# servo/webrender

Measured on AMD Instinct MI355X. Metric: frames/sec + Mpixels/sec on wrench benchmarks, 4K target, 1/2/4/8 GPU, higher is better.
Workload: dtype u8; 1 GPU; cfg2: 1000 overlapping translucent rects (ps_quad_textured + premultiplied-alpha blend), 3840x2160, 20 picture-cache tiles + composite, seed 2; encoding=quad, target=3840x2160, parallelism=single GPU

## Files before the change

include/wrhip.h:

```cpp
#ifndef WRHIP_H
#define WRHIP_H

#include <stddef.h>
#include <stdint.h>

#ifdef __cplusplus
extern "C" {
#endif

typedef int8_t GLbyte;
typedef uint8_t GLubyte;
typedef int16_t GLshort;
typedef uint16_t GLushort;
typedef int32_t GLint;
typedef uint32_t GLuint;
typedef int64_t GLint64;
typedef uint64_t GLuint64;
typedef float GLfloat;
typedef double GLdouble;
typedef uint32_t GLenum;
typedef uint8_t GLboolean;
typedef uint32_t GLbitfield;
typedef int32_t GLsizei;
typedef size_t GLsizeiptr;
// ... 97 lines not shown
                GLenum ty, void* data);
void Finish(void);
void ShaderSourceByName(GLuint shader, const GLchar* name);
void TexParameteri(GLenum target, GLenum pname, GLint param);
void CopyImageSubData(GLuint src_name, GLenum src_target, GLint src_level,
                      GLint src_x, GLint src_y, GLint src_z, GLuint dst_name,
                      GLenum dst_target, GLint dst_level, GLint dst_x,
                      GLint dst_y, GLint dst_z, GLsizei src_width,
                      GLsizei src_height, GLsizei src_depth);
void CopyTexSubImage2D(GLenum target, GLint level, GLint xoffset, GLint yoffset,
                       GLint x, GLint y, GLsizei width,
                       GLsizei height);
void BlitFramebuffer(GLint src_x0, GLint src_y0, GLint src_x1, GLint src_y1,
                     GLint dst_x0, GLint dst_y0, GLint dst_x1, GLint dst_y1,
                     GLbitfield mask, GLenum filter);
void GetIntegerv(GLenum pname, GLint* params);
void GetBooleanv(GLenum pname, GLboolean* params);
const char* GetString(GLenum name);
const char* GetStringi(GLenum name, GLuint index);
GLenum GetError(void);
void InitDefaultFramebuffer(int32_t x, int32_t y, int32_t width, int32_t height,
                            int32_t stride, void* buf);
void* GetColorBuffer(GLuint fbo, GLboolean flush, int32_t* width,
                     int32_t* height, int32_t* stride);
void ResolveFramebuffer(GLuint fbo);
void SetTextureBuffer(GLuint tex, GLenum internal_format, GLsizei width,
                      GLsizei height, GLsizei stride, void* buf,
                      GLsizei min_width, GLsizei min_height);
void SetTextureParameter(GLuint tex, GLenum pname, GLint param);
void DeleteTexture(GLuint n);
void DeleteRenderbuffer(GLuint n);
void DeleteFramebuffer(GLuint n);
void DeleteBuffer(GLuint n);
void DeleteVertexArray(GLuint n);
void DeleteQuery(GLuint n);
void DeleteShader(GLuint shader);
void DeleteProgram(GLuint program);
LockedTexture* LockFramebuffer(GLuint fbo);
LockedTexture* LockTexture(GLuint tex);
void LockResource(LockedTexture* resource);
void UnlockResource(LockedTexture* resource);
void* GetResourceBuffer(LockedTexture* resource, int32_t* width,
                        int32_t* height, int32_t* stride);
void Composite(LockedTexture* locked_dst, LockedTexture* locked_src, GLint src_x,
               GLint src_y, GLsizei src_width, GLsizei src_height, GLint dst_x,
               GLint dst_y, GLsizei dst_width, GLsizei dst_height,
               GLboolean opaque, GLboolean flip_x, GLboolean flip_y,
               GLenum filter, GLint clip_x, GLint clip_y, GLsizei clip_width,
               GLsizei clip_height);
void CompositeYUV(LockedTexture* locked_dst, LockedTexture* locked_y,
                  LockedTexture* locked_u, LockedTexture* locked_v,
                  YuvRangedColorSpace color_space, GLuint color_depth,
                  GLint src_x, GLint src_y, GLsizei src_width,
                  GLsizei src_height, GLint dst_x, GLint dst_y,
                  GLsizei dst_width, GLsizei dst_height, GLboolean flip_x,
                  GLboolean flip_y, GLint clip_x, GLint clip_y,
                  GLsizei clip_width, GLsizei clip_height);
WrhipContext* CreateContext(void);
void ReferenceContext(WrhipContext* ctx);
void DestroyContext(WrhipContext* ctx);
void MakeCurrent(WrhipContext* ctx);
size_t ReportMemory(WrhipContext* ctx,
                    size_t (*size_of_op)(const void* ptr));


typedef struct WrhipStats {
  uint64_t flushes;
  uint64_t kernel_launches;
  uint64_t raster_launches;
  uint64_t raster_ns;
  uint64_t raster_algo_bytes;
  uint64_t raster_pixels;
  uint64_t prims;
  uint64_t h2d_bytes;
  uint64_t d2h_bytes;
  uint64_t host_record_ns;
  uint64_t host_upload_ns;
  uint64_t host_flush_ns;
  uint64_t host_wait_ns;
  uint64_t row_launches;
  uint64_t setup_carried;
  uint64_t carrier_lost;
  uint64_t scratch_grown_held;
} WrhipStats;
void WrhipGetStats(WrhipStats* out);
void WrhipResetStats(void);
void WrhipSetProfiling(int enabled);
typedef struct WrhipKernelStat {
  int32_t kind, fmt, depth, feat;
  uint64_t launches, ns, algo_bytes, workgroups;
} WrhipKernelStat;
int32_t WrhipGetKernelStats(WrhipKernelStat* out, int32_t max);
void WrhipSetShard(int rank, int world);
void WrhipSetTargetRows(GLuint tex, int32_t y0, int32_t y1);
void* WrhipGetTextureDevicePtr(GLuint tex, int32_t* width, int32_t* height,
                               int32_t* stride);
GLuint WrhipGetFramebufferTexture(GLuint fbo);
const char* WrhipDeviceName(void);
void WrhipFlush(void);
int WrhipFlushHeld(void);
void* WrhipGetStream(void);

#ifdef __cplusplus
}
#endif
#endif
```

webrender_amd/csrc/wrhip.hip:

```cpp
#include <vector>
#include <map>
#include <algorithm>
#include <time.h>
#include <chrono>
#include <thread>
#include <pthread.h>
#include <mutex>
#include <condition_variable>
#include <atomic>
#include <functional>

#include "../../include/wrhip.h"
#include "wrhip_glenum.h"
#include "wrhip_types.h"
#include "wrhip_rt.h"
#include "wrhip_kernels.h"
#ifndef WRHIP_HOSTSIM
#include "wrhip_inst.h"
#define WR_INST_DECLARE(K, SIG, ...) extern template __global__ void K<__VA_ARGS__> SIG;
WR_INST_ALL(WR_INST_DECLARE)
#undef WR_INST_DECLARE
#endif

namespace {
// ... 325 lines not shown
  int sampler_unit[WR_MAX_TEX];
  float transform[16];
  Program() {
    for (int& a : attrib_loc) a = NULL_ATTRIB;
    for (int& s : sampler_unit) s = 0;
    memset(transform, 0, sizeof(transform));
  }
};

struct TargetWork {
  GLuint tex = 0;
  GLuint depth_tex = 0;
  std::vector<WrDrawDesc> draws;
  std::vector<uint8_t> inst;
  std::vector<GLuint> reads;
  std::vector<GLuint> rreads;
  int prims = 0;
  int level = 0;
  uint32_t init_depth = 0xFFFFFF;
  bool init_depth_set = false, depth_live = false;
  GLuint fwd_tex = 0; int fwd_dx = 0, fwd_y0 = 0, fwd_ys = 1, fwd_clip[4] = {0, 0, 0, 0};
  bool forwarded_away = false;
  void recycle() {
    std::vector<WrDrawDesc> d; d.swap(draws); d.clear();
    std::vector<uint8_t> i; i.swap(inst); i.clear();
    std::vector<GLuint> r; r.swap(reads); r.clear();
    std::vector<GLuint> rr; rr.swap(rreads); rr.clear();
    *this = TargetWork();
    draws.swap(d); inst.swap(i); reads.swap(r); rreads.swap(rr);
  }
};

const size_t MAX_TEXTURE_UNITS = 16;

struct Context {
  int32_t references = 1;
  ObjectStore<Query> queries;
  ObjectStore<Buffer> buffers;
  ObjectStore<Texture> textures;
  ObjectStore<VertexArray> vertex_arrays;
  ObjectStore<Framebuffer> framebuffers;
  ObjectStore<Renderbuffer> renderbuffers;
  ObjectStore<Shader> shaders;
  ObjectStore<Program> programs;

  GLenum last_error = GL_NO_ERROR;
  int viewport[4] = {0, 0, 0, 0};
  bool blend = false;
  GLenum blendfunc_srgb = GL_ONE, blendfunc_drgb = GL_ZERO, blendfunc_sa = GL_ONE, blendfunc_da = GL_ZERO;
  GLenum blend_equation = GL_FUNC_ADD;
  uint32_t blendcolor[2] = {0, 0};
  int blend_key = WR_BLEND_NONE;
  bool depthtest = false, depthmask = true;
  GLenum depthfunc = GL_LESS;
  bool scissortest = false;
  int scissor[4] = {0, 0, 0, 0};
  float clearcolor[4] = {0, 0, 0, 0};
  double cleardepth = 1;
  int unpack_row_length = 0;

  struct TextureUnit { GLuint texture_2d_binding = 0, texture_rectangle_binding = 0; };
  TextureUnit texture_units[MAX_TEXTURE_UNITS];
  int active_texture_unit = 0;
  GLuint current_program = 0, current_vertex_array = 0;
  GLuint pixel_pack_buffer_binding = 0, pixel_unpack_buffer_binding = 0, array_buffer_binding = 0;
  GLuint time_elapsed_query = 0, samples_passed_query = 0;
  GLuint renderbuffer_binding = 0, draw_framebuffer_binding = 0, read_framebuffer_binding = 0;
  GLuint unknown_binding = 0;

  wr_stream_t stream;
  std::vector<TargetWork> work;
  std::vector<TargetWork> spare;
  std::vector<GLuint> referenced;
  struct UploadSeg { uint64_t src_off; void* dst; uint32_t dst_stride, row_bytes, rows, pad; };
  std::vector<UploadSeg> useg;
  size_t upload_begin = 0;
  bool upload_open = false;
  uint64_t lap_ns[8] = {0, 0, 0, 0, 0, 0, 0, 0}; uint64_t lap_n = 0;
  uint64_t upload_batch = 1;
  bool scatter_first = false;
  std::vector<GLuint> view_texs;
  struct PendingScatter { size_t seg_off = 0; int nseg = 0, parts = 0; uint64_t bytes = 0; bool valid = false; } ps;
  bool fuse_scatter = true;
  uint8_t* dupload = nullptr;
  struct Scratch {
    WrPrim* prims = nullptr; size_t prims_cap = 0;
    WrRec* recs = nullptr;
    WrAux* aux = nullptr;
    float* vtab = nullptr; size_t vtab_cap = 0;
    float* qtab = nullptr; size_t qtab_cap = 0;
    unsigned long long* masks = nullptr; size_t masks_cap = 0;
    unsigned* bin_ctr = nullptr; size_t bin_ctr_cap = 0;
    unsigned long long* mr_ctl = nullptr; WrMaskSlot* mr_slots = nullptr; size_t mr_slots_cap = 0;
    uint8_t* mr_store = nullptr; size_t mr_store_cap = 0;
    unsigned long long mr_seen = 0;
    uint32_t* flat = nullptr; size_t flat_cap = 0;
  } scratch[2];
  int64_t flush_seq = 0;
  int64_t held_seq = 0;
  int fb_writes_since_held = 0;
  bool last_flush_wrote_fb = false;
  struct Held { int fmt, depth, feat, nb, off; uint64_t algo_bytes; int mr_rows = 0; int dense = 0; int row_t0 = 0, row_n = 0, row_items = 0, row_mode = 0; };
  struct Tail {
    bool pending = false;
    std::vector<Held> held;
    int n_targets = 0;
    const WrTargetDesc* targets = nullptr; const WrDrawDesc* draws = nullptr;
    int set = 0;
    std::vector<GLuint> refs;
  } tail;
  bool defer_tail = true;
  wr_stream_t copy_stream;
  wr_event_t ev_copy;
  bool copy_overlap = true;
  wr_stream_t setup_stream;
  wr_event_t ev_up, ev_setup;
  bool setup_on_stream = false;
  WrUnsupportedCounters* dcounters = nullptr;
  WrUnsupportedCounters seen = {};
  std::multimap<size_t, void*> pool;
  size_t pool_bytes = 0;
  uint8_t* staging = nullptr; size_t staging_size = 0, staging_pos = 0;
  uint64_t ring_base = 0, ring_safe = 0;
  struct RingFence { uint64_t v = 0; wr_event_t ev; bool made = false; };
  static const int RING_FENCES = 8;
  RingFence ring_fence[RING_FENCES];
  uint64_t ring_fences = 0;
  bool profiling = false;
  bool profiling_deferred = false;
  wr_event_t ev_a, ev_b;
  WrhipStats stats;
  std::vector<WrhipKernelStat> kstats;
  int shard_rank = 0, shard_world = 1;
  int next_query_slot = 0;
  GLuint query_slot_owner[WR_QUERY_SLOTS] = {};
  bool forward_composites = true;
  bool profiling_no_forward = false;
  bool mask_rows = true;
  bool span_rows = true;
  bool tile_rows = true;
  bool grad_tables = true;
  size_t gtab_pending = 0;
  bool quad_rowtabs = true;
  size_t runs_pool_words = (size_t)16 << 20;
  unsigned long long* last_qctl = nullptr;
  size_t last_qtab_cap = 0;
  uint64_t last_qctl_v = 0;
  bool cell_raster = true;
  bool thin_r8 = true;
  int thin_parts = 4;
  bool dense_text = false;
  int chain_grid = 0;
  unsigned chain_base = 0;

  Context() {
    wrrt::stream_create(&stream);
    wrrt::stream_create(&copy_stream);
    wrrt::event_create_sync(&ev_copy);
    wrrt::stream_create(&setup_stream);
    wrrt::event_create_sync(&ev_up);
    wrrt::event_create_sync(&ev_setup);
    setup_on_stream = getenv("WRHIP_SETUP_STREAM") && atoi(getenv("WRHIP_SETUP_STREAM")) != 0;
    copy_overlap = getenv("WRHIP_NO_COPY_STREAM") == nullptr;
    forward_composites = getenv("WRHIP_NO_FORWARD") == nullptr;
    thin_r8 = getenv("WRHIP_NO_THIN") == nullptr;
    if (const char* e = getenv("WRHIP_THIN_PARTS")) { const int v = atoi(e); if (v == 1 || v == 2 || v == 4 || v == 8 || v == 16) thin_parts = v; }
    dense_text = getenv("WRHIP_DENSE_TEXT") != nullptr;
    if (thin_r8 && getenv("WRHIP_CHAIN") && atoi(getenv("WRHIP_CHAIN")) > 0)
      chain_grid = getenv("WRHIP_CHAIN_GRID") ? atoi(getenv("WRHIP_CHAIN_GRID")) : wrrt::cu_count() / 2;
    cell_raster = getenv("WRHIP_NO_CELLS") == nullptr;
    fuse_scatter = getenv("WRHIP_NO_FUSE_SCATTER") == nullptr;
    mask_rows = getenv("WRHIP_NO_MASK_ROWS") == nullptr;
    span_rows = getenv("WRHIP_NO_SPAN_ROWS") == nullptr;
    tile_rows = getenv("WRHIP_NO_TILE_ROWS") == nullptr;
    quad_rowtabs = getenv("WRHIP_NO_QTAB") == nullptr;
    grad_tables = getenv("WRHIP_NO_GTAB") == nullptr;
    if (const char* e = getenv("WRHIP_RUNS_POOL_WORDS")) runs_pool_words = (size_t)atoll(e);
    wrrt::event_create(&ev_a); wrrt::event_create(&ev_b);
    memset(&stats, 0, sizeof(stats));
    dcounters = (WrUnsupportedCounters*)wrrt::dev_alloc(sizeof(WrUnsupportedCounters));
    wrrt::memset8(dcounters, 0, sizeof(WrUnsupportedCounters), stream);
  }
  ~Context();

  GLuint& get_binding(GLenum name) {
    switch (name) {
      case GL_PIXEL_PACK_BUFFER: return pixel_pack_buffer_binding;
      case GL_PIXEL_UNPACK_BUFFER: return pixel_unpack_buffer_binding;
      case GL_ARRAY_BUFFER: return array_buffer_binding;
      case GL_ELEMENT_ARRAY_BUFFER: return vertex_arrays[current_vertex_array].element_array_buffer_binding;
      case GL_TEXTURE_2D: return texture_units[active_texture_unit].texture_2d_binding;
      case GL_TEXTURE_RECTANGLE: return texture_units[active_texture_unit].texture_rectangle_binding;
      case GL_TIME_ELAPSED: return time_elapsed_query;
      case GL_SAMPLES_PASSED: return samples_passed_query;
      case GL_RENDERBUFFER: return renderbuffer_binding;
      case GL_DRAW_FRAMEBUFFER: return draw_framebuffer_binding;
      case GL_READ_FRAMEBUFFER: return read_framebuffer_binding;
      default: return unknown_binding;
    }
  }
};

Context* ctx = nullptr;
bool g_rt_ok = false, g_rt_tried = false;
char g_device_name[256] = "";

void ensure_runtime() {
  if (g_rt_tried) {
    if (!g_rt_ok) { fprintf(stderr, "libwrhip: no HIP device available; this backend has no CPU path\n"); abort(); }
    return;
  }
  g_rt_tried = true;
  int dev = 0;
  g_rt_ok = wrrt::init(&dev, g_device_name, sizeof(g_device_name));
  if (!g_rt_ok) { fprintf(stderr, "libwrhip: no HIP device available; this backend has no CPU path\n"); abort(); }
}

int bytes_for_internal_format(GLenum f) {
  switch (f) {
    case GL_RGBA32F: case GL_RGBA32I: return 16;
    case GL_RGBA8: case GL_BGRA8: case GL_RGBA: return 4;
    case GL_R8: case GL_RED: return 1;
    case GL_RG8: case GL_RG: return 2;
    case GL_DEPTH_COMPONENT: case GL_DEPTH_COMPONENT16: case GL_DEPTH_COMPONENT24: case GL_DEPTH_COMPONENT32: return 4;
    case GL_RGB_RAW_422_APPLE: return 2;
    case GL_R16: return 2;
    case GL_RG16: return 4;
    default: return 0;
  }
}
int aligned_stride(int row_bytes) { return (row_bytes + 3) & ~3; }
GLenum remap_internal_format(GLenum format) {
  switch (format) {
    case GL_DEPTH_COMPONENT: return GL_DEPTH_COMPONENT24;
    case GL_RGBA: return GL_RGBA8;
    case GL_RED: return GL_R8;
    case GL_RG: return GL_RG8;
    case GL_RGB_422_APPLE: return GL_RGB_RAW_422_APPLE;
    default: return format;
  }
}
int wr_format(GLenum f) {
  switch (f) {
    case GL_RGBA32F: return WR_FMT_RGBA32F;
    case GL_RGBA32I: return WR_FMT_RGBA32I;
    case GL_RGBA8: return WR_FMT_RGBA8;
    case GL_R8: return WR_FMT_R8;
    case GL_RG8: return WR_FMT_RG8;
    case GL_R16: return WR_FMT_R16;
    case GL_RG16: return WR_FMT_RG16;
    case GL_DEPTH_COMPONENT24: return WR_FMT_DEPTH24;
    default: return WR_FMT_NONE;
  }
}
// ... 427 lines not shown
  d.clear_color = color_value;
  d.clear_depth = depth_value;
  for (int k = 0; k < WR_MAX_ATTRIBS; k++) d.attr_off[k] = -1;
  TargetWork& w = ctx->work[wi];
  if (depth) {
    w.depth_tex = depth_tex;
    Texture& dt = ctx->textures[depth_tex];
    if (!w.init_depth_set) { w.init_depth = dt.depth_value; w.init_depth_set = true; }
    w.depth_live = true;
    dt.depth_owner = tex_id;
  }
  w.draws.push_back(d);
  w.prims += 1;
}

void download_texture(Texture& t) {
  sync_texture_for_read(t);
  if (!t.dptr) return;
  size_t row = (size_t)t.bpp * t.width;
  if (t.ext_buf) {
    wrrt::copy2d(t.ext_buf, t.ext_stride, t.dptr, t.stride, row, t.height, 1, ctx->stream);
  } else {
    size_t need = (size_t)t.stride * t.height;
    if (t.hmirror_size < need) { free(t.hmirror); t.hmirror = (uint8_t*)malloc(need + 64); t.hmirror_size = need; }
    wrrt::copy2d(t.hmirror, t.stride, t.dptr, t.stride, row, t.height, 1, ctx->stream);
  }
  ctx->stats.d2h_bytes += row * t.height;
  sync_stream();
}

Context::~Context() {
  Context* saved = ctx;
  ctx = this;
  flush_all();
  flush_uploads(1206);
  sync_stream();
  for (Texture* t : textures.objects) if (t) { if (t->dptr) wrrt::dev_free(t->dptr); t->dptr = nullptr; free(t->hmirror); t->hmirror = nullptr; }
  for (auto& kv : pool) wrrt::dev_free(kv.second);
  pool.clear();
  wrrt::dev_free(dupload); wrrt::dev_free(dcounters);
  for (Scratch& S : scratch) { wrrt::dev_free(S.prims); wrrt::dev_free(S.recs); wrrt::dev_free(S.aux); wrrt::dev_free(S.vtab); wrrt::dev_free(S.qtab); wrrt::dev_free(S.masks); wrrt::dev_free(S.bin_ctr); wrrt::dev_free(S.mr_slots); wrrt::dev_free(S.mr_store); wrrt::dev_free(S.flat); }
  wrrt::pinned_free(staging);
  wrrt::event_destroy(ev_a); wrrt::event_destroy(ev_b);
  wrrt::event_destroy(ev_copy);
  for (RingFence& f : ring_fence) if (f.made) wrrt::event_destroy(f.ev);
  wrrt::stream_destroy(copy_stream);
  wrrt::stream_destroy(stream);
  ctx = saved == this ? nullptr : saved;
}

void prof_begin(wr_stream_t* on) { if (ctx->profiling) wrrt::event_record(&ctx->ev_a, on ? *on : ctx->stream); }
void prof_end(int kind, int fmt, int depth, int feat, uint64_t algo_bytes, uint64_t workgroups, wr_stream_t* on) {
  Context* c = ctx;
  if (!c->profiling) return;
  wrrt::event_record(&c->ev_b, on ? *on : c->stream);
  wrrt::event_sync(&c->ev_b);
  const uint64_t ns = (uint64_t)(wrrt::event_elapsed_ms(&c->ev_a, &c->ev_b) * 1.0e6);
  WrhipKernelStat* k = nullptr;
  for (WrhipKernelStat& e : c->kstats) if (e.kind == kind && e.fmt == fmt && e.depth == depth && e.feat == feat) k = &e;
  if (!k) { c->kstats.push_back(WrhipKernelStat{kind, fmt, depth, feat, 0, 0, 0, 0}); k = &c->kstats.back(); }
  k->launches++; k->ns += ns; k->algo_bytes += algo_bytes; k->workgroups += workgroups;
  if (kind == 2 || kind == 4 || kind == 5 || kind == 6 || kind == 7 || kind == 9 || kind == 10 || kind == 11 || kind == 12 || kind == 13) c->stats.raster_ns += ns;
}

void tail_launched() {
  Context::Tail& T = ctx->tail;
  for (GLuint id : T.refs) if (Texture* t = ctx->textures.find(id)) t->tail_ref = false;
  T.refs.clear();
  T.held.clear();
  T.pending = false;
}
#ifndef WR_THIN_MAX_BINS
#define WR_THIN_MAX_BINS 256
#endif
bool can_fuse(const Context::Held& H) {
  if (H.row_n > 0) return H.row_mode == 2;
  if (H.mr_rows > 0) return true;
  static const bool thin_first = getenv("WRHIP_FUSE_SMALL") == nullptr;
  static const bool fuse_thin = getenv("WRHIP_NO_FUSE_THIN") == nullptr;
  if (thin_first && ctx->thin_r8 && H.fmt == WR_FMT_RGBA8 && !H.depth && H.nb <= WR_THIN_MAX_BINS && H.feat == (WR_FEAT_TEX | WR_FEAT_GENERIC)) return fuse_thin;
  return H.fmt == WR_FMT_RGBA8 && (H.feat == 0 || H.feat == (WR_FEAT_TEX | WR_FEAT_GENERIC) ||
                                   H.feat == (WR_FEAT_TEX | WR_FEAT_GENERIC | WR_FEAT_R8TEX));
}
bool chainable(const Context::Held& H) {
  return ctx->chain_grid > 0 && H.row_n == 0 && H.fmt == WR_FMT_R8 && H.nb <= WR_THIN_MAX_BINS && (H.feat == 0 || H.feat == (WR_FEAT_GENERIC | WR_FEAT_BLUR));
}
void launch_raster(const Context::Held& H, const WrTargetDesc* targets, int n_targets, const WrDrawDesc* draws, Context::Scratch& S,
                   const WrSetupArgs* SA = nullptr, int n_setup_blocks = 0, int chain_n = 1, uint64_t setup_bytes = 0) {
  Context* c = ctx;
#define WR_K(FMT, DEPTH, FEAT)                                                                                          \
  do {                                                                                                                  \
    WR_LAUNCH((wr_raster_kernel<FMT, DEPTH, 4, FEAT>), H.nb, 256, c->stream, targets, n_targets, draws,                 \
              (const WrPrim*)S.prims, (const WrRec*)S.recs, (const WrAux*)S.aux, (const float*)S.vtab, S.masks, H.off); \
  } while (0)
#define WR_KF(DEPTH, FEAT)                                                                                              \
  do {                                                                                                                  \
    WR_LAUNCH((wr_setup_raster_kernel<WR_FMT_RGBA8, DEPTH, 4, FEAT>), n_setup_blocks + SA->up_blocks + H.nb, 256, c->stream, *SA,        \
              n_setup_blocks, targets, n_targets, draws, (const WrPrim*)S.prims, (const WrRec*)S.recs,                  \
              (const WrAux*)S.aux, (const float*)S.vtab, S.masks, H.off);                                               \
  } while (0)
  if (H.row_n > 0) {
    const int wgs = std::max(1, std::min((H.row_items + 3) / 4, 16384));
    static const bool dbg_rows = getenv("WRHIP_DEBUG_ROWS") != nullptr;
    if (dbg_rows) fprintf(stderr, "span rows (mode %d): targets [%d, %d) items %d workgroups %d\n", H.row_mode, H.row_t0, H.row_t0 + H.row_n, H.row_items, wgs);
    prof_begin();
    const bool rows_fused = SA != nullptr && H.row_mode == 2;
    if (rows_fused) WR_LAUNCH(wr_setup_tile_rows_kernel, n_setup_blocks + SA->up_blocks + wgs, 256, c->stream, *SA, n_setup_blocks, targets, H.row_t0, H.row_n, draws, (const WrPrim*)S.prims, (const WrAux*)S.aux);
    else if (H.row_mode == 2) WR_LAUNCH(wr_tile_rows_kernel, wgs, 256, c->stream, targets, H.row_t0, H.row_n, draws, (const WrPrim*)S.prims, (const WrAux*)S.aux);
    else WR_LAUNCH(wr_span_rows_kernel, wgs, 256, c->stream, targets, H.row_t0, H.row_n, draws, (const WrPrim*)S.prims, (const WrAux*)S.aux);
    prof_end(rows_fused ? 11 : (H.row_mode == 2 ? 10 : 9), H.fmt, 0, 0, H.algo_bytes + (rows_fused ? setup_bytes : 0), (uint64_t)wgs + (rows_fused ? n_setup_blocks : 0));
    c->stats.kernel_launches++; c->stats.raster_launches++; c->stats.row_launches++;
    return;
  }
  const int F5 = WR_FEAT_TEX | WR_FEAT_GENERIC, F7 = F5 | WR_FEAT_R8TEX, FA = F7 | WR_FEAT_BLUR | WR_FEAT_SHADE;
  if (H.mr_rows > 0 && S.mr_ctl) {
    const int wgs = std::max(1, std::min((H.mr_rows + 3) / 4, 4096));
    prof_begin();
    const bool rows_fused = SA != nullptr;
    if (SA) {
      WR_LAUNCH(wr_setup_rows_kernel, n_setup_blocks + SA->up_blocks + wgs, 256, c->stream, *SA, n_setup_blocks, targets, H.off, H.off + H.nb,
                (const WrPrim*)S.prims, (const WrAux*)S.aux, S.mr_ctl, (const WrMaskSlot*)S.mr_slots, S.mr_store);
      SA = nullptr;
    } else
    WR_LAUNCH(wr_mask_rows_kernel, wgs, 256, c->stream, targets, H.off, H.off + H.nb, (const WrPrim*)S.prims, (const WrAux*)S.aux,
              S.mr_ctl, (const WrMaskSlot*)S.mr_slots, S.mr_store);
    prof_end(rows_fused ? 8 : 3, H.fmt, 0, 0, rows_fused ? setup_bytes : 0, (uint64_t)wgs + (rows_fused ? n_setup_blocks : 0));
    if (c->profiling) {
      unsigned long long parts[32], seen = 0;
      wrrt::d2h(parts, S.mr_ctl + 32, sizeof(parts), c->stream);
      wrrt::stream_sync(c->stream);
      for (unsigned long long v : parts) seen += v;
      for (WrhipKernelStat& e : c->kstats) if (e.kind == (rows_fused ? 8 : 3) && e.fmt == H.fmt) e.algo_bytes += seen - S.mr_seen;
      S.mr_seen = seen;
    }
    c->stats.kernel_launches++;
  }
  if (chain_n >= 2) {
    WrChain ch;
    memset(&ch, 0, sizeof(ch));
    ch.n = chain_n;
    int widest = 0; uint64_t bytes = 0;
    for (int i = 0; i < chain_n; i++) { ch.first[i] = (&H)[i].off; ch.count[i] = (&H)[i].nb; widest = std::max(widest, (&H)[i].nb); bytes += (&H)[i].algo_bytes; }
    const int grid = std::max(1, std::min(widest, c->chain_grid));
    for (int l = 0; l + 1 < chain_n; l++) {
      int part = 0;
      for (int k = l; k < chain_n; k++) part = std::max(part, std::min(grid, ch.count[k]));
      c->chain_base += (unsigned)part;
      ch.want[l] = c->chain_base;
    }
    prof_begin();
    if (H.feat == 0)
      WR_LAUNCH((wr_raster_chain_kernel<0>), grid, 1024, c->stream, targets, n_targets, draws, (const WrPrim*)S.prims, (const WrRec*)S.recs,
                (const WrAux*)S.aux, (const float*)S.vtab, S.masks, ch, &c->dcounters->chain_arrive, c->dcounters);
    else
      WR_LAUNCH((wr_raster_chain_kernel<WR_FEAT_GENERIC | WR_FEAT_BLUR>), grid, 1024, c->stream, targets, n_targets, draws, (const WrPrim*)S.prims,
                (const WrRec*)S.recs, (const WrAux*)S.aux, (const float*)S.vtab, S.masks, ch, &c->dcounters->chain_arrive, c->dcounters);
    prof_end(4, H.fmt, chain_n, H.feat, bytes, (uint64_t)grid);
    c->stats.kernel_launches++; c->stats.raster_launches++;
    return;
  }
  prof_begin();
  uint64_t thin_wgs = 0;
  const bool fused = SA != nullptr;
  static const bool thin_carrier = getenv("WRHIP_FUSE_SMALL") == nullptr;
  if (H.dense && H.fmt == WR_FMT_RGBA8 && H.feat == F7) {
#define WR_KD(DEPTH)                                                                                                         \
  do {                                                                                                                       \
    if (SA) WR_LAUNCH((wr_setup_raster_dense_kernel<WR_FMT_RGBA8, DEPTH, 4, WR_FEAT_TEX | WR_FEAT_GENERIC | WR_FEAT_R8TEX>), \
                      n_setup_blocks + SA->up_blocks + H.nb, 256, c->stream, *SA, n_setup_blocks, targets, n_targets, draws,                 \
                      (const WrPrim*)S.prims, (const WrRec*)S.recs, (const WrAux*)S.aux, (const float*)S.vtab, S.masks, H.off); \
    else WR_LAUNCH((wr_raster_dense_kernel<WR_FMT_RGBA8, DEPTH, 4, WR_FEAT_TEX | WR_FEAT_GENERIC | WR_FEAT_R8TEX>), H.nb, 256, \
                   c->stream, targets, n_targets, draws, (const WrPrim*)S.prims, (const WrRec*)S.recs, (const WrAux*)S.aux,  \
                   (const float*)S.vtab, S.masks, H.off);                                                                    \
  } while (0)
    if (H.depth) WR_KD(true); else WR_KD(false);
#undef WR_KD
  }
  else if (SA && H.fmt == WR_FMT_RGBA8 && !H.depth && c->thin_r8 && H.nb <= WR_THIN_MAX_BINS && H.feat == F5 && thin_carrier) {
    thin_wgs = (uint64_t)H.nb * 4 + (uint64_t)n_setup_blocks;
    WR_LAUNCH((wr_setup_raster_thin_kernel<WR_FMT_RGBA8, false, 1, WR_FEAT_TEX | WR_FEAT_GENERIC>), n_setup_blocks + SA->up_blocks + H.nb * 4, 256, c->stream, *SA,
              n_setup_blocks, targets, n_targets, draws, (const WrPrim*)S.prims, (const WrRec*)S.recs, (const WrAux*)S.aux, (const float*)S.vtab, S.masks, H.off);
  }
  else if (SA) {
    if (H.depth) {
      if (H.feat == 0) WR_KF(true, 0); else if (H.feat == F5) WR_KF(true, WR_FEAT_TEX | WR_FEAT_GENERIC);
      else WR_KF(true, WR_FEAT_TEX | WR_FEAT_GENERIC | WR_FEAT_R8TEX);
    } else {
      if (H.feat == 0) WR_KF(false, 0); else if (H.feat == F5) WR_KF(false, WR_FEAT_TEX | WR_FEAT_GENERIC);
      else WR_KF(false, WR_FEAT_TEX | WR_FEAT_GENERIC | WR_FEAT_R8TEX);
    }
  }
  else if (H.fmt == WR_FMT_RGBA8 && !H.depth && c->thin_r8 && H.nb <= WR_THIN_MAX_BINS && H.feat != 0 && H.feat != F7) {
    thin_wgs = (uint64_t)H.nb * 4;
    if (H.feat == F5)
      WR_LAUNCH((wr_raster_kernel<WR_FMT_RGBA8, false, 1, WR_FEAT_TEX | WR_FEAT_GENERIC>), H.nb * 4, 256, c->stream, targets, n_targets, draws,
                (const WrPrim*)S.prims, (const WrRec*)S.recs, (const WrAux*)S.aux, (const float*)S.vtab, S.masks, H.off);
    else
      WR_LAUNCH((wr_raster_kernel<WR_FMT_RGBA8, false, 1, WR_FEAT_TEX | WR_FEAT_GENERIC | WR_FEAT_R8TEX | WR_FEAT_BLUR | WR_FEAT_SHADE>), H.nb * 4, 256, c->stream,
                targets, n_targets, draws, (const WrPrim*)S.prims, (const WrRec*)S.recs, (const WrAux*)S.aux, (const float*)S.vtab, S.masks, H.off);
  }
  else if (H.fmt == WR_FMT_RGBA8) {
    if (H.depth) {
      if (H.feat == 0) WR_K(WR_FMT_RGBA8, true, 0); else if (H.feat == F5) WR_K(WR_FMT_RGBA8, true, WR_FEAT_TEX | WR_FEAT_GENERIC);
      else if (H.feat == F7) WR_K(WR_FMT_RGBA8, true, WR_FEAT_TEX | WR_FEAT_GENERIC | WR_FEAT_R8TEX);
      else WR_K(WR_FMT_RGBA8, true, WR_FEAT_TEX | WR_FEAT_GENERIC | WR_FEAT_R8TEX | WR_FEAT_BLUR | WR_FEAT_SHADE);
    } else {
      if (H.feat == 0) WR_K(WR_FMT_RGBA8, false, 0); else if (H.feat == F5) WR_K(WR_FMT_RGBA8, false, WR_FEAT_TEX | WR_FEAT_GENERIC);
      else if (H.feat == F7) WR_K(WR_FMT_RGBA8, false, WR_FEAT_TEX | WR_FEAT_GENERIC | WR_FEAT_R8TEX);
      else WR_K(WR_FMT_RGBA8, false, WR_FEAT_TEX | WR_FEAT_GENERIC | WR_FEAT_R8TEX | WR_FEAT_BLUR | WR_FEAT_SHADE);
    }
    (void)FA;
  } else {
    const bool thin = c->thin_r8 && H.nb <= WR_THIN_MAX_BINS;
    if (thin && (H.feat == 0 || H.feat == (WR_FEAT_GENERIC | WR_FEAT_BLUR))) thin_wgs = (uint64_t)H.nb * c->thin_parts;
#define WR_K1(FEAT)                                                                                                     \
  do {                                                                                                                  \
    WR_LAUNCH((wr_raster_kernel<WR_FMT_R8, false, 1, FEAT>), H.nb * c->thin_parts, 1024 / c->thin_parts, c->stream, targets, n_targets, draws,          \
              (const WrPrim*)S.prims, (const WrRec*)S.recs, (const WrAux*)S.aux, (const float*)S.vtab, S.masks, H.off); \
  } while (0)
    if (H.feat == 0) { if (thin) WR_K1(0); else WR_K(WR_FMT_R8, false, 0); }
    else if (H.feat == (WR_FEAT_GENERIC | WR_FEAT_BLUR)) { if (thin) WR_K1(WR_FEAT_GENERIC | WR_FEAT_BLUR); else WR_K(WR_FMT_R8, false, WR_FEAT_GENERIC | WR_FEAT_BLUR); }
    else WR_K(WR_FMT_R8, false, WR_FEAT_GENERIC | WR_FEAT_BLUR | WR_FEAT_CLIP);
#undef WR_K1
  }
#undef WR_K
#undef WR_KF
  prof_end(thin_wgs ? (fused ? 13 : 12) : fused ? (H.dense ? 7 : 6) : (H.dense ? 5 : 2), H.fmt, H.depth, H.feat, H.algo_bytes + (fused ? setup_bytes : 0),
           thin_wgs ? thin_wgs : (uint64_t)H.nb + (fused ? n_setup_blocks : 0));
  c->stats.kernel_launches++; c->stats.raster_launches++;
}
void launch_held(const std::vector<Context::Held>& held, const WrTargetDesc* targets, int n_targets, const WrDrawDesc* draws, Context::Scratch& S,
                 int fuse_at = -1, const WrSetupArgs* SA = nullptr, int n_setup_blocks = 0, uint64_t setup_bytes = 0) {
  for (size_t i = 0; i < held.size();) {
    size_t j = i + 1;
    if (chainable(held[i]) && !(S.mr_ctl == nullptr && held[i].mr_rows > 0))
      while (j < held.size() && j - i < WR_MAX_CHAIN && chainable(held[j]) && held[j].feat == held[i].feat && held[j].mr_rows == 0 && (int)j != fuse_at) j++;
    const bool fuse = (int)i == fuse_at;
    launch_raster(held[i], targets, n_targets, draws, S, fuse ? SA : nullptr, fuse ? n_setup_blocks : 0, (int)(j - i), fuse ? setup_bytes : 0);
    i = j;
  }
}
void drain_tail() {
  Context* c = ctx;
  if (!c || !c->tail.pending) return;
  Context::Tail& T = c->tail;
  launch_held(T.held, T.targets, T.n_targets, T.draws, c->scratch[T.set]);
  tail_launched();
}
void sync_stream() {
  drain_tail();
  HostTimer ht(&ctx->stats.host_wait_ns);
  wrrt::stream_sync(ctx->stream);
}
void sync_scratch() {
  if (ctx->tail.pending) ctx->stats.scratch_grown_held++;
  HostTimer ht(&ctx->stats.host_wait_ns);
  wrrt::stream_sync(ctx->stream);
}

static bool plan_forwarding(TargetWork& fb, const std::vector<int>& sel) {
  Context* c = ctx;
  Texture& ft = c->textures[fb.tex];
  if (ft.internal_format != GL_RGBA8 || c->profiling_no_forward) return false;
  const bool strip = ft.own_y1 > ft.own_y0;
  const int oy0 = strip ? std::max(0, ft.own_y0) : 0, oy1 = strip ? std::min(ft.height, ft.own_y1) : ft.height;
  if (oy1 <= oy0) return false;
  struct Plan { int src; int dx, y0, ys, clip[4]; };
  std::vector<Plan> plans;
  bool seen_draw = false;
  for (const WrDrawDesc& d : fb.draws) {
    if (d.shader == WR_SH_CLEAR_OP) {
      const bool full = d.clip[0] <= 0 && d.clip[1] <= 0 && d.clip[2] >= ft.width && d.clip[3] >= ft.height;
      if (seen_draw || !full || (d.flags & WR_DF_CLEAR_DEPTH)) return false;
      continue;
    }
    seen_draw = true;
    if (d.shader != WR_SH_COMPOSITE_FAST || d.blend != WR_BLEND_NONE || (d.flags & (WR_DF_DEPTH_TEST | WR_DF_DEPTH_WRITE | WR_DF_TEX_RECT)) || d.query_slot >= 0) return false;
    if (d.attr_off[0] < 0 || d.attr_off[1] < 0 || d.attr_off[4] < 0 || d.attr_bytes[0] < 16 || d.attr_bytes[1] < 16 || d.attr_bytes[4] < 16) return false;
    if (d.quad[0] != 0.f || d.quad[1] != 0.f || d.quad[2] != 1.f || d.quad[3] != 0.f || d.quad[4] != 1.f || d.quad[5] != 1.f || d.quad[6] != 0.f || d.quad[7] != 1.f) return false;
    const WrTexDesc& st = d.tex[WR_S_COLOR0];
    if (!st.ptr || st.format != WR_FMT_RGBA8) return false;
    int src = -1;
    for (int wi : sel) if (&c->work[wi] != &fb && c->textures[c->work[wi].tex].dptr == st.ptr && c->work[wi].level < fb.level && !c->work[wi].forwarded_away) src = wi;
    if (src < 0 && !strip) return false;
    if (src >= 0 && c->work[src].fwd_tex && c->work[src].fwd_tex != fb.tex) return false;
    for (int i = 0; i < d.count; i++) {
      const uint8_t* ip = fb.inst.data() + d.inst_offset + (size_t)i * d.inst_stride;
      float rect[4], clip[4], prm[4] = {0, 0, 0, 0}, uv[4], flip[2] = {0, 0};
      memcpy(rect, ip + d.attr_off[0], 16); memcpy(clip, ip + d.attr_off[1], 16); memcpy(uv, ip + d.attr_off[4], 16);
      if (d.attr_off[3] >= 0 && d.attr_bytes[3] >= 16) memcpy(prm, ip + d.attr_off[3], 16);
      if (d.attr_off[5] >= 0 && d.attr_bytes[5] >= 8) memcpy(flip, ip + d.attr_off[5], 8);
      if (flip[0] != 0.f || flip[1] != 0.f || int(prm[1]) == 1 || uv[0] != 0.f || uv[1] != 0.f || uv[2] != 1.f || uv[3] != 1.f) return false;
      auto to_px = [&](float x, float y, float& sx, float& sy) {
        const float* m = d.transform;
        const float gx = m[0] * x + m[4] * y + m[12], gy = m[1] * x + m[5] * y + m[13], gw = m[3] * x + m[7] * y + m[15];
        sx = (gx / gw + 1.0f) * 0.5f * d.vp_size[0] + d.vp_origin[0];
        sy = (gy / gw + 1.0f) * 0.5f * d.vp_size[1] + d.vp_origin[1];
      };
      if (d.transform[1] != 0.f || d.transform[4] != 0.f || d.transform[3] != 0.f || d.transform[7] != 0.f) return false;
      float x0, y0, x1, y1, cx0, cy0, cx1, cy1;
      to_px(rect[0], rect[1], x0, y0); to_px(rect[2], rect[3], x1, y1);
      to_px(clip[0], clip[1], cx0, cy0); to_px(clip[2], clip[3], cx1, cy1);
      auto near_int = [](float v, int& o) { o = (int)lrintf(v); return fabsf(v - (float)o) < 1.0f / 64.0f; };
      int ix0, iy0, ix1, iy1, icx0, icy0, icx1, icy1;
      if (!near_int(x0, ix0) || !near_int(y0, iy0) || !near_int(x1, ix1) || !near_int(y1, iy1) || !near_int(cx0, icx0) || !near_int(cy0, icy0) ||
          !near_int(cx1, icx1) || !near_int(cy1, icy1)) return false;
      if (strip && std::min(std::max(icy0, icy1), oy1) <= std::max(std::min(icy0, icy1), oy0)) continue;
      if (strip && std::min(std::max(iy0, iy1), oy1) <= std::max(std::min(iy0, iy1), oy0)) continue;
      if (src < 0) return false;
      const Texture& stex = c->textures[c->work[src].tex];
      if (ix1 - ix0 != stex.width || abs(iy1 - iy0) != stex.height) return false;
      for (const Plan& q : plans) if (q.src == src) return false;
      Plan P;
      P.src = src; P.dx = ix0;
      if (iy1 > iy0) { P.y0 = iy0; P.ys = 1; } else { P.y0 = iy0 - 1; P.ys = -1; }
      P.clip[0] = std::max(std::max(std::min(icx0, icx1), d.clip[0]), std::max(0, std::min(ix0, ix1)));
      P.clip[1] = std::max(std::max(std::min(icy0, icy1), d.clip[1]), std::max(0, std::min(iy0, iy1)));
      P.clip[2] = std::min(std::min(std::max(icx0, icx1), d.clip[2]), std::min(ft.width, std::max(ix0, ix1)));
      P.clip[3] = std::min(std::min(std::max(icy0, icy1), d.clip[3]), std::min(ft.height, std::max(iy0, iy1)));
      if (P.clip[2] <= P.clip[0] || P.clip[3] <= P.clip[1]) { P.clip[0] = P.clip[1] = P.clip[2] = P.clip[3] = 0; }
      plans.push_back(P);
// ... 343 lines not shown
      T.mr_max_slots = (uint32_t)S.mr_slots_cap;
    }
  }
  for (WrTargetDesc& T : targets) { T.flat_rows = nullptr; T.counters = c->dcounters; }
  static const bool no_flat = getenv("WRHIP_NO_FLAT") != nullptr;
  if (flat_words && any_work && !no_flat) {
    Context::Scratch& S = c->scratch[c->flush_seq & 1];
    if (S.flat_cap < flat_words) {
      sync_scratch();
      wrrt::dev_free(S.flat);
      S.flat_cap = flat_words * 2;
      S.flat = (uint32_t*)wrrt::dev_alloc(S.flat_cap * 4);
    }
    wrrt::memset8(S.flat, 0xFF, flat_words * 4, c->stream);
    for (int oi = 0; oi < n_targets; oi++) if (flat_off[oi] != SIZE_MAX) targets[oi].flat_rows = S.flat + flat_off[oi];
  }
  if (any_work) {
    lap(0);
    size_t off_draws = 0;
    size_t off_targets = (off_draws + sizeof(WrDrawDesc) * nd + 255) & ~size_t(255);
    size_t off_inst = (off_targets + sizeof(WrTargetDesc) * n_targets + 255) & ~size_t(255);
    const int n_blocks = (n_prims + 63) / 64;
    size_t off_blk = (off_inst + inst_bytes + 255) & ~size_t(255);
    const size_t off_qctl = (off_blk + sizeof(WrBlock) * n_blocks + 63) & ~size_t(63);
    const size_t off_mrctl = off_qctl + 64;
    size_t total = off_mrctl + 512 + 256;
    size_t aoff = staging_alloc(total);
    uint8_t* h = c->staging + aoff;
    for (GLuint id : c->view_texs) {
      Texture* t = c->textures.find(id);
      if (!t || !t->dptr || !c->upload_open || t->view_batch != c->upload_batch) continue;
      const void* view = c->dupload + t->view_off;
      for (WrDrawDesc& d : draws)
        for (WrTexDesc& td : d.tex) if (td.ptr == t->dptr) td.ptr = view;
    }
    c->view_texs.clear();
    memset(h + off_qctl, 0, 64 + 512);
    if (mr_on) {
      Context::Scratch& Sm = c->scratch[c->flush_seq & 1];
      Sm.mr_ctl = (unsigned long long*)(c->dupload + aoff + off_mrctl); Sm.mr_seen = 0;
      for (WrTargetDesc& T : targets) if (T.format == WR_FMT_R8 && T.mr_slots) T.mr_ctl = Sm.mr_ctl;
    }
    *(unsigned long long*)(h + off_qctl) = (unsigned long long)gtab_words;
    for (WrTargetDesc& T : targets) T.qtab_ctl = T.qtab ? (unsigned long long*)(c->dupload + aoff + off_qctl) : nullptr;
    c->last_qctl = nullptr;
    for (const WrTargetDesc& T : targets) if (T.qtab) { c->last_qctl = T.qtab_ctl; c->last_qtab_cap = T.qtab_cap; c->last_qctl_v = c->ring_base + aoff + off_qctl; break; }
    if (nd) stage_copy(h + off_draws, draws.data(), sizeof(WrDrawDesc) * nd);
    stage_copy(h + off_targets, targets.data(), sizeof(WrTargetDesc) * n_targets);
    if (inst_bytes >= PARALLEL_COPY_MIN && inst_segs.size() > 1) {
      copy_pool().run([&](int part, int parts) {
        for (size_t i = (size_t)part; i < inst_segs.size(); i += (size_t)parts) stage_copy(h + off_inst + inst_segs[i].base, inst_segs[i].src, inst_segs[i].size);
      });
    } else {
      for (const InstSeg& sg : inst_segs) {
        if (sg.size >= PARALLEL_COPY_MIN) big_memcpy(h + off_inst + sg.base, sg.src, sg.size);
        else stage_copy(h + off_inst + sg.base, sg.src, sg.size);
      }
    }
    {
      WrBlock* blk = (WrBlock*)(h + off_blk);
      int j = 0;
      for (int b = 0; b < n_blocks; b++) {
        while (j + 1 < nd && draws[j + 1].first_prim <= 64 * b) j++;
        WrBlock B;
        B.lo0 = j; B.nk = nd - j >= 2 ? 2 : nd - j;
        B.t0 = B.nk > 0 ? draws[j].target : -1; B.t1 = B.nk > 1 ? draws[j + 1].target : -1;
        blk[b] = B;
      }
    }
    int fuse_at = -1;
    if (n_prims > 0 && c->tail.pending && !c->setup_on_stream) {
      int best_rows = 0;
      for (size_t hi = 0; hi < c->tail.held.size(); hi++)
        if (c->tail.held[hi].mr_rows > best_rows) { best_rows = c->tail.held[hi].mr_rows; fuse_at = (int)hi; }
      if (fuse_at < 0) {
        int best_items = 0;
        for (size_t hi = 0; hi < c->tail.held.size(); hi++) {
          const Context::Held& Hh = c->tail.held[hi];
          if (Hh.row_n > 0 && Hh.row_mode == 2 && Hh.row_items > best_items && can_fuse(Hh)) { best_items = Hh.row_items; fuse_at = (int)hi; }
        }
      }
      for (size_t hi = 0; hi < c->tail.held.size() && fuse_at < 0; hi++) if (can_fuse(c->tail.held[hi])) fuse_at = (int)hi;
    }
    lap(1);
    flush_uploads(0, fuse_at >= 0);
    uint8_t* darena = c->dupload + aoff;
    c->stats.h2d_bytes += total;
    algo_bytes += inst_bytes + sizeof(WrDrawDesc) * nd;
    lap(2);
    Context::Scratch& S = c->scratch[c->flush_seq & 1];
#ifdef WRHIP_HOSTSIM
    wrrt::memset8(S.masks, 0, (size_t)n_words * 8, c->stream);
#endif
    const WrDrawDesc* ddraws = (const WrDrawDesc*)(darena + off_draws);
    const WrTargetDesc* dtargets = (const WrTargetDesc*)(darena + off_targets);
    const uint8_t* dinst = darena + off_inst;
    const int* dblk = (const int*)(darena + off_blk);
    if (n_prims > 0) {
#ifdef WRHIP_TIMING
      static const int setup_mode = getenv("WRHIP_SETUP_MODE") ? atoi(getenv("WRHIP_SETUP_MODE")) : 0;
      const int nd_arg = nd | (setup_mode << 24);
#else
      const int nd_arg = nd;
#endif
      const int n_setup_blocks = (n_prims + 255) / 256;
      const uint64_t setup_bytes = inst_bytes + sizeof(WrDrawDesc) * nd + (uint64_t)n_prims * (sizeof(WrPrim) + sizeof(WrRec));
      if (c->tail.pending && c->setup_on_stream) {
        wrrt::event_record(&c->ev_up, c->stream);
        wrrt::stream_wait_event(c->setup_stream, &c->ev_up);
        prof_begin(&c->setup_stream);
        WR_LAUNCH(wr_setup_kernel, n_setup_blocks, 256, c->setup_stream, ddraws, nd_arg, dinst, S.prims, S.recs, S.aux, n_prims,
                  dtargets, S.masks, S.vtab, c->dcounters, dblk);
        prof_end(1, 0, 0, 0, setup_bytes, (uint64_t)n_setup_blocks, &c->setup_stream);
        wrrt::event_record(&c->ev_setup, c->setup_stream);
        c->stats.kernel_launches += 1;
        drain_tail();
        wrrt::stream_wait_event(c->stream, &c->ev_setup);
      } else {
      if (fuse_at >= 0 && !(c->tail.pending && fuse_at < (int)c->tail.held.size())) {
        c->stats.carrier_lost++;
        fuse_at = -1;
      }
      if (fuse_at >= 0) {
        Context::Tail& T = c->tail;
        WrSetupArgs SA{ddraws, nd_arg, dinst, S.prims, S.recs, S.aux, n_prims, dtargets, S.masks, S.vtab, c->dcounters, dblk, nullptr, 0, 0, 0};
        uint64_t carried = setup_bytes;
        if (c->ps.valid) {
          SA.up_segs = (const WrUploadSeg*)(c->dupload + c->ps.seg_off); SA.up_nseg = c->ps.nseg; SA.up_parts = c->ps.parts; SA.up_blocks = c->ps.nseg * c->ps.parts;
          carried += c->ps.bytes;
          c->ps.valid = false;
        }
        c->stats.setup_carried++;
        launch_held(T.held, T.targets, T.n_targets, T.draws, c->scratch[T.set], fuse_at, &SA, n_setup_blocks, carried);
        tail_launched();
      } else {
        launch_pending_scatter();
        prof_begin();
        WR_LAUNCH(wr_setup_kernel, n_setup_blocks, 256, c->stream, ddraws, nd_arg, dinst, S.prims, S.recs, S.aux, n_prims,
                  dtargets, S.masks, S.vtab, c->dcounters, dblk);
        prof_end(1, 0, 0, 0, setup_bytes, (uint64_t)n_setup_blocks);
        c->stats.kernel_launches += 1;
        drain_tail();
      }
      }
    } else {
      drain_tail();
    }
    launch_pending_scatter();
    lap(3);
#ifdef WRHIP_HOSTSIM
    if (getenv("WRHIP_DEBUG")) {
      fprintf(stderr, "flush: targets %d draws %d prims %d bins %d words %d vtab %zu set %d carried %llu grown_held %llu\n", n_targets, nd, n_prims, n_bins,
              n_words, vtab_cursor, (int)(c->flush_seq & 1), (unsigned long long)c->stats.setup_carried, (unsigned long long)c->stats.scratch_grown_held);
      for (int i = 0; i < n_targets; i++)
        fprintf(stderr, "  T%d %dx%d fmt %d load %d init %08x prims [%d,%d) wpb %d\n", i, targets[i].width, targets[i].height,
                targets[i].format, targets[i].load_color, targets[i].init_color, targets[i].first_prim, targets[i].end_prim,
                targets[i].words_per_bin);
      for (int i = 0; i < nd && i < 6; i++)
        fprintf(stderr, "  D%d sh %d tgt %d first %d n %d blend %d flags %x clip %d %d %d %d vp %g %g %g %g\n", i, draws[i].shader,
                draws[i].target, draws[i].first_prim, draws[i].count, draws[i].blend, draws[i].flags, draws[i].clip[0],
                draws[i].clip[1], draws[i].clip[2], draws[i].clip[3], draws[i].vp_origin[0], draws[i].vp_origin[1],
                draws[i].vp_size[0], draws[i].vp_size[1]);
      for (int i = 0; i < nd && i < 6; i++)
        fprintf(stderr, "     inst off %llu stride %d attr_off %d %d %d %d %d %d bytes %d %d quad %g %g %g %g %g %g %g %g\n",
                (unsigned long long)draws[i].inst_offset, draws[i].inst_stride, draws[i].attr_off[0], draws[i].attr_off[1],
                draws[i].attr_off[2], draws[i].attr_off[3], draws[i].attr_off[4], draws[i].attr_off[5], draws[i].attr_bytes[0],
                draws[i].attr_bytes[1], draws[i].quad[0], draws[i].quad[1], draws[i].quad[2], draws[i].quad[3], draws[i].quad[4],
                draws[i].quad[5], draws[i].quad[6], draws[i].quad[7]);
      for (int i = 0; i < nd && i < 6; i++) {
        const float* f = (const float*)(dinst + draws[i].inst_offset);
        fprintf(stderr, "     flush inst D%d: %g %g %g %g (inst bytes %zu)\n", i, f[0], f[1], f[2], f[3], inst_bytes);
      }
      for (int i = 0; i < n_prims && i < 6; i++) {
        const WrPrim& P = S.prims[i];
        fprintf(stderr, "  P%d kind %d rect %d %d %d %d z %u blend %d flags %x color %08x %08x\n", i, P.kind, P.x0, P.y0, P.x1, P.y1,
                P.z, P.blend, P.flags, P.color[0], P.color[1]);
      }
    }
#endif
    for (int i = 0; i < nd; i++) {
      if (targets[draws[i].target].rows_mode) continue;
      const bool to_r8 = targets[draws[i].target].format == WR_FMT_R8;
      Level& L = levels[target_level[draws[i].target]];
      int f = 0;
      if (!(draws[i].flags & WR_DF_SIMPLE)) {
        switch (draws[i].shader) {
          case WR_SH_PS_CLEAR: case WR_SH_CLEAR_OP: break;
          case WR_SH_PS_TEXT_RUN: case WR_SH_PS_TEXT_RUN_DUAL: case WR_SH_PS_TEXT_RUN_GT: case WR_SH_PS_TEXT_RUN_DUAL_GT: f = WR_FEAT_R8TEX | WR_FEAT_TEX | WR_FEAT_GENERIC; break;
          case WR_SH_BRUSH_SOLID: case WR_SH_BRUSH_SOLID_ALPHA: f = WR_FEAT_R8TEX | WR_FEAT_GENERIC; break;
          case WR_SH_CS_BLUR_ALPHA: case WR_SH_CS_BLUR_COLOR: f = WR_FEAT_BLUR; break;
          case WR_SH_CS_CLIP_RECT: case WR_SH_CS_CLIP_RECT_FAST: case WR_SH_CS_CLIP_BOX_SHADOW:
            f = ((draws[i].flags & WR_DF_MASK_ROWS) && mr_safe) ? WR_FEAT_BLUR : WR_FEAT_CLIP; break;
          case WR_SH_BRUSH_LINEAR_GRADIENT: case WR_SH_BRUSH_LINEAR_GRADIENT_ALPHA: case WR_SH_CS_LINEAR_GRADIENT: case WR_SH_CS_RADIAL_GRADIENT: case WR_SH_CS_CONIC_GRADIENT: f = WR_FEAT_SHADE | WR_FEAT_GENERIC; break;
          case WR_SH_BRUSH_BLEND: case WR_SH_BRUSH_BLEND_ALPHA: f = WR_FEAT_SHADE | WR_FEAT_GENERIC; break;
          case WR_SH_BRUSH_MIX_BLEND: case WR_SH_BRUSH_MIX_BLEND_ALPHA: f = WR_FEAT_SHADE | WR_FEAT_GENERIC; break;
          case WR_SH_CS_SVG_FILTER: case WR_SH_CS_SVG_FILTER_NODE: f = WR_FEAT_SHADE | WR_FEAT_GENERIC; break;
          case WR_SH_BRUSH_YUV: case WR_SH_BRUSH_YUV_ALPHA: case WR_SH_COMPOSITE_YUV: f = WR_FEAT_SHADE | WR_FEAT_GENERIC; break;
          case WR_SH_PS_QUAD_MASK: case WR_SH_PS_QUAD_MASK_FAST: case WR_SH_PS_QUAD_RADIAL_GRADIENT: case WR_SH_PS_QUAD_CONIC_GRADIENT:
            f = WR_FEAT_SHADE | WR_FEAT_GENERIC; break;
          case WR_SH_CS_BORDER_SOLID: case WR_SH_CS_BORDER_SEGMENT: case WR_SH_CS_FAST_LINEAR_GRADIENT: case WR_SH_CS_LINE_DECORATION:
            f = WR_FEAT_SHADE | WR_FEAT_GENERIC; break;
          case WR_SH_BRUSH_IMAGE_REPEAT: case WR_SH_BRUSH_IMAGE_REPEAT_ALPHA: case WR_SH_BRUSH_IMAGE_REPEAT_DUAL: f = WR_FEAT_SHADE | WR_FEAT_GENERIC; break;
          default: f = WR_FEAT_TEX | WR_FEAT_GENERIC; break;
        }
      }
      if (draws[i].flags & WR_DF_QUADS) f |= WR_FEAT_SHADE | WR_FEAT_GENERIC;
      (to_r8 ? L.feat_r8 : L.feat_rgba) |= f;
      if (!to_r8 && !(draws[i].flags & WR_DF_SIMPLE) && (draws[i].shader == WR_SH_PS_TEXT_RUN || draws[i].shader == WR_SH_PS_TEXT_RUN_DUAL || draws[i].shader == WR_SH_PS_TEXT_RUN_GT || draws[i].shader == WR_SH_PS_TEXT_RUN_DUAL_GT)) L.text = true;
    }
    std::vector<Context::Held> launches;
    for (const Level& L : levels) {
      if (L.bins_rgba > 0) {
        int f;
        if (L.feat_rgba == 0) f = 0;
        else if (!(L.feat_rgba & ~(WR_FEAT_TEX | WR_FEAT_GENERIC))) f = WR_FEAT_TEX | WR_FEAT_GENERIC;
        else if (!(L.feat_rgba & ~(WR_FEAT_TEX | WR_FEAT_GENERIC | WR_FEAT_R8TEX))) f = WR_FEAT_TEX | WR_FEAT_GENERIC | WR_FEAT_R8TEX;
// ... 1371 lines not shown
```

webrender_amd/csrc/wrhip_inst.h:

```cpp
#pragma once
#define WR_SIG_PLAIN (const WrTargetDesc*, int, const WrDrawDesc*, const WrPrim*, const WrRec*, const WrAux*, const float*, unsigned long long*, int)
#define WR_SIG_FUSED (WrSetupArgs, int, const WrTargetDesc*, int, const WrDrawDesc*, const WrPrim*, const WrRec*, const WrAux*, const float*, unsigned long long*, int)
#define WR_INST_1(X) X(wr_raster_kernel, WR_SIG_PLAIN, WR_FMT_RGBA8, true, 4, 47)
#define WR_INST_2(X) X(wr_raster_kernel, WR_SIG_PLAIN, WR_FMT_RGBA8, false, 4, 47)
#define WR_INST_3(X)                                                                                                          \
  X(wr_raster_kernel, WR_SIG_PLAIN, WR_FMT_RGBA8, true, 4, 7) X(wr_raster_kernel, WR_SIG_PLAIN, WR_FMT_RGBA8, false, 4, 7)    \
  X(wr_raster_kernel, WR_SIG_PLAIN, WR_FMT_RGBA8, true, 4, 5) X(wr_raster_kernel, WR_SIG_PLAIN, WR_FMT_RGBA8, false, 4, 5)    \
  X(wr_raster_kernel, WR_SIG_PLAIN, WR_FMT_RGBA8, true, 4, 0) X(wr_raster_kernel, WR_SIG_PLAIN, WR_FMT_RGBA8, false, 4, 0)
#define WR_INST_4(X)                                                                                                                      \
  X(wr_setup_raster_kernel, WR_SIG_FUSED, WR_FMT_RGBA8, true, 4, 7) X(wr_setup_raster_kernel, WR_SIG_FUSED, WR_FMT_RGBA8, false, 4, 7)    \
  X(wr_setup_raster_kernel, WR_SIG_FUSED, WR_FMT_RGBA8, true, 4, 5) X(wr_setup_raster_kernel, WR_SIG_FUSED, WR_FMT_RGBA8, false, 4, 5)    \
  X(wr_setup_raster_kernel, WR_SIG_FUSED, WR_FMT_RGBA8, true, 4, 0) X(wr_setup_raster_kernel, WR_SIG_FUSED, WR_FMT_RGBA8, false, 4, 0)
#define WR_INST_5(X)                                                                                                                            \
  X(wr_raster_dense_kernel, WR_SIG_PLAIN, WR_FMT_RGBA8, true, 4, 7) X(wr_raster_dense_kernel, WR_SIG_PLAIN, WR_FMT_RGBA8, false, 4, 7)          \
  X(wr_setup_raster_dense_kernel, WR_SIG_FUSED, WR_FMT_RGBA8, true, 4, 7) X(wr_setup_raster_dense_kernel, WR_SIG_FUSED, WR_FMT_RGBA8, false, 4, 7)
#define WR_INST_6(X)                                                                                                  \
  X(wr_raster_kernel, WR_SIG_PLAIN, WR_FMT_R8, false, 4, 0) X(wr_raster_kernel, WR_SIG_PLAIN, WR_FMT_R8, false, 4, 12) \
  X(wr_raster_kernel, WR_SIG_PLAIN, WR_FMT_R8, false, 4, 28)
#define WR_INST_7(X) X(wr_raster_kernel, WR_SIG_PLAIN, WR_FMT_RGBA8, false, 1, 5) X(wr_raster_kernel, WR_SIG_PLAIN, WR_FMT_RGBA8, false, 1, 47)
#define WR_INST_8(X) X(wr_setup_raster_thin_kernel, WR_SIG_FUSED, WR_FMT_RGBA8, false, 1, 5)
#define WR_INST_ALL(X) WR_INST_1(X) WR_INST_2(X) WR_INST_3(X) WR_INST_4(X) WR_INST_5(X) WR_INST_6(X) WR_INST_7(X) WR_INST_8(X)
#define WR_INST_GROUPS 8
```

webrender_amd/csrc/wrhip_k_raster.h:

```cpp
#pragma once

WR_DEVICE bool wr_kind_needs_runs(int kind) {
  return kind == WR_PK_TEX_RGBA8 || kind == WR_PK_TEX_R8 || kind == WR_PK_TEX_FS || kind == WR_PK_GRADIENT || kind == WR_PK_FILTER || kind == WR_PK_MIX_BLEND || kind == WR_PK_SVG_FILTER || kind == WR_PK_YUV || kind == WR_PK_QUAD_MASK || kind == WR_PK_BORDER_SOLID || kind == WR_PK_BORDER_SEGMENT || kind == WR_PK_FAST_GRADIENT || kind == WR_PK_LINE_DECORATION ||
         kind == WR_PK_TEX_REPEAT || kind == WR_PK_TEX_QUAD || kind == WR_PK_SOLID_QUAD || kind == WR_PK_SOLID_AA;
}
WR_DEVICE void wr_occ_interval(const WrRec* __restrict__ recs, const WrAux* __restrict__ aux, int ci, int y, int& lo, int& hi) {
  const WrRec Rc = recs[ci];
  lo = hi = 0;
  if (y < Rc.y0 || y >= Rc.y1) return;
  const int kind = Rc.kbf & 0xFF;
  if (kind == WR_PK_SOLID_QUAD || kind == WR_PK_TEX_QUAD) {
    int s0, s1;
    if (wr_quad_row_span(aux[ci].quad, y, s0, s1) && s1 > s0) { lo = wr_imax(s0, Rc.x0); hi = wr_imin(s1, Rc.x1); if (hi < lo) hi = lo; }
    return;
  }
  lo = Rc.x0; hi = Rc.x1;
}
template <typename IV>
WR_DEVICE int wr_sweep_into(WrRuns& R, int32_t* ext, int a, int b, int nc, IV iv) {
  int n = 0, pos = a;
  while (pos < b) {
    int s = pos;
    for (bool moved = true; moved;) {
      moved = false;
// ... 1610 lines not shown
                 const WrDrawDesc* __restrict__ draws, const WrPrim* __restrict__ prims,
                 const WrRec* __restrict__ recs, const WrAux* __restrict__ aux, const float* __restrict__ vtab,
                 unsigned long long* __restrict__ masks, int bin_offset) {
  if constexpr (R == 1) {
    const int parts = 1024 / (int)blockDim.x;
    wr_raster_body<FMT, DEPTH, R, FEAT>(targets, n_targets, draws, prims, recs, aux, vtab, masks, (int)blockIdx.x / parts + bin_offset, (int)blockIdx.x % parts, parts);
  } else
  wr_raster_body<FMT, DEPTH, R, FEAT>(targets, n_targets, draws, prims, recs, aux, vtab, masks, (int)blockIdx.x + bin_offset);
}

struct WrChain { int n; int first[WR_MAX_CHAIN]; int count[WR_MAX_CHAIN]; unsigned want[WR_MAX_CHAIN]; };
template <int FEAT>
__global__ void __launch_bounds__(1024)
wr_raster_chain_kernel(const WrTargetDesc* __restrict__ targets, int n_targets,
                       const WrDrawDesc* __restrict__ draws, const WrPrim* __restrict__ prims,
                       const WrRec* __restrict__ recs, const WrAux* __restrict__ aux, const float* __restrict__ vtab,
                       unsigned long long* __restrict__ masks, WrChain ch, unsigned* __restrict__ arrive,
                       WrUnsupportedCounters* __restrict__ cnt) {
#ifndef WRHIP_HOSTSIM
  for (int l = 0; l < ch.n; l++) {
    for (int b = (int)blockIdx.x; b < ch.count[l]; b += (int)gridDim.x) {
      wr_raster_body<WR_FMT_R8, false, 1, FEAT>(targets, n_targets, draws, prims, recs, aux, vtab, masks, ch.first[l] + b);
      __syncthreads();
    }
    if (l + 1 == ch.n) break;
    bool more = false;
    for (int k = l + 1; k < ch.n; k++) more = more || (int)blockIdx.x < ch.count[k];
    __syncthreads();
    if (threadIdx.x == 0) {
      const unsigned want = ch.want[l];
      __builtin_amdgcn_fence(__ATOMIC_RELEASE, "agent");
      __hip_atomic_fetch_add(arrive, 1u, __ATOMIC_RELAXED, __HIP_MEMORY_SCOPE_AGENT);
      unsigned spins = 0;
      while (more && (int)(__hip_atomic_load(arrive, __ATOMIC_RELAXED, __HIP_MEMORY_SCOPE_AGENT) - want) < 0) {
        __builtin_amdgcn_s_sleep(8);
        if (++spins > (1u << 21)) { atomicAdd(&cnt->chain_timeout, 1u); break; }
      }
      if (more) __builtin_amdgcn_fence(__ATOMIC_ACQUIRE, "agent");
    }
    if (!more) return;
    __syncthreads();
  }
#endif
}

#if defined(WR_SETUP_PRIORITY) && !defined(WRHIP_HOSTSIM)
#define WR_SETUP_PRIO() __builtin_amdgcn_s_setprio(WR_SETUP_PRIORITY)
#else
#define WR_SETUP_PRIO() ((void)0)
#endif
struct WrSetupArgs {
  const WrDrawDesc* draws; int n_draws; const uint8_t* arena; WrPrim* prims; WrRec* recs; WrAux* aux; int n_prims;
  const WrTargetDesc* targets; unsigned long long* masks; float* vtab; WrUnsupportedCounters* cnt; const int* blk;
  const WrUploadSeg* up_segs; int up_nseg, up_parts, up_blocks;
};
#define WR_FUSED_PROLOGUE(S, n_setup_blocks)                                                                                      \
  int wr_bid = (int)blockIdx.x;                                                                                                   \
  if (wr_bid < (S).up_blocks) { wr_upload_body((S).up_segs, (S).up_nseg, (S).up_parts, wr_bid); return; }                         \
  wr_bid -= (S).up_blocks;                                                                                                        \
  if (wr_bid < (n_setup_blocks)) {                                                                                                \
    WR_SETUP_PRIO();                                                                                                              \
    wr_setup_body((S).draws, (S).n_draws, (S).arena, (S).prims, (S).recs, (S).aux, (S).n_prims, (S).targets, (S).masks, (S).vtab, (S).cnt, (S).blk, wr_bid); \
    return;                                                                                                                       \
  }                                                                                                                               \
  wr_bid -= (n_setup_blocks);
#ifdef WRHIP_HOSTSIM
#define WR_FUSED_BOUNDS(R, FEAT) __launch_bounds__(1024 / R)
#else
#ifndef WR_FUSED_RECT_WAVES
#define WR_FUSED_RECT_WAVES 4
#endif
#define WR_FUSED_BOUNDS(R, FEAT) __launch_bounds__(1024 / R, (FEAT) == 0 ? WR_FUSED_RECT_WAVES : WR_TEX_WAVES)
#endif
template <int FMT, bool DEPTH, int R, int FEAT>
__global__ void WR_FUSED_BOUNDS(R, FEAT)
wr_setup_raster_kernel(WrSetupArgs S, int n_setup_blocks,
                       const WrTargetDesc* __restrict__ targets, int n_targets,
                       const WrDrawDesc* __restrict__ draws, const WrPrim* __restrict__ prims,
                       const WrRec* __restrict__ recs, const WrAux* __restrict__ aux, const float* __restrict__ vtab,
                       unsigned long long* __restrict__ masks, int bin_offset) {
  WR_FUSED_PROLOGUE(S, n_setup_blocks)
  wr_raster_body<FMT, DEPTH, R, FEAT>(targets, n_targets, draws, prims, recs, aux, vtab, masks, wr_bid + bin_offset);
}
template <int FMT, bool DEPTH, int R, int FEAT>
__global__ void __launch_bounds__(256, WR_TEX_WAVES)
wr_setup_raster_thin_kernel(WrSetupArgs S, int n_setup_blocks,
                            const WrTargetDesc* __restrict__ targets, int n_targets,
                            const WrDrawDesc* __restrict__ draws, const WrPrim* __restrict__ prims,
                            const WrRec* __restrict__ recs, const WrAux* __restrict__ aux, const float* __restrict__ vtab,
                            unsigned long long* __restrict__ masks, int bin_offset) {
  static_assert(R == 1 && FMT == WR_FMT_RGBA8 && !DEPTH, "the thin colour shape");
  WR_FUSED_PROLOGUE(S, n_setup_blocks)
  const int b = wr_bid;
  wr_raster_body<FMT, DEPTH, R, FEAT>(targets, n_targets, draws, prims, recs, aux, vtab, masks, b / 4 + bin_offset, b % 4, 4);
}
#ifndef WR_DENSE_WAVES
#define WR_DENSE_WAVES 4
#endif
template <int FMT, bool DEPTH, int R, int FEAT>
__global__ void __launch_bounds__(1024 / R, WR_DENSE_WAVES)
wr_raster_dense_kernel(const WrTargetDesc* __restrict__ targets, int n_targets,
                       const WrDrawDesc* __restrict__ draws, const WrPrim* __restrict__ prims,
                       const WrRec* __restrict__ recs, const WrAux* __restrict__ aux, const float* __restrict__ vtab,
                       unsigned long long* __restrict__ masks, int bin_offset) {
  wr_raster_body<FMT, DEPTH, R, FEAT>(targets, n_targets, draws, prims, recs, aux, vtab, masks, (int)blockIdx.x + bin_offset);
}
template <int FMT, bool DEPTH, int R, int FEAT>
__global__ void __launch_bounds__(1024 / R, WR_DENSE_WAVES)
wr_setup_raster_dense_kernel(WrSetupArgs S, int n_setup_blocks,
                             const WrTargetDesc* __restrict__ targets, int n_targets,
                             const WrDrawDesc* __restrict__ draws, const WrPrim* __restrict__ prims,
                             const WrRec* __restrict__ recs, const WrAux* __restrict__ aux, const float* __restrict__ vtab,
                             unsigned long long* __restrict__ masks, int bin_offset) {
  WR_FUSED_PROLOGUE(S, n_setup_blocks)
  wr_raster_body<FMT, DEPTH, R, FEAT>(targets, n_targets, draws, prims, recs, aux, vtab, masks, wr_bid + bin_offset);
}
#ifndef WR_INST_ONLY
__global__ void __launch_bounds__(256, 4)
wr_setup_rows_kernel(WrSetupArgs S, int n_setup_blocks, const WrTargetDesc* __restrict__ targets, int bin_lo, int bin_hi,
                     const WrPrim* __restrict__ prims, const WrAux* __restrict__ aux, unsigned long long* __restrict__ ctl,
                     const WrMaskSlot* __restrict__ slots, uint8_t* __restrict__ store) {
  WR_FUSED_PROLOGUE(S, n_setup_blocks)
  wr_mask_rows_body(targets, bin_lo, bin_hi, prims, aux, ctl, slots, store, wr_bid, (int)gridDim.x - n_setup_blocks - S.up_blocks);
}
__global__ void __launch_bounds__(256, 4)
wr_setup_tile_rows_kernel(WrSetupArgs S, int n_setup_blocks, const WrTargetDesc* __restrict__ targets, int t0, int nt, const WrDrawDesc* __restrict__ draws,
                          const WrPrim* __restrict__ prims, const WrAux* __restrict__ aux) {
  WR_FUSED_PROLOGUE(S, n_setup_blocks)
  wr_tile_rows_body(targets, t0, nt, draws, prims, aux, wr_bid, (int)gridDim.x - n_setup_blocks - S.up_blocks);
}
#endif
```

webrender_amd/csrc/wrhip_k_setup.h:

```cpp
#pragma once

#ifndef WR_DEVICE
#define WR_DEVICE __device__ __forceinline__
#endif

#ifdef WRHIP_HOSTSIM
static unsigned long long wr_dbg_paths[8];
#define WR_DBG_PATH(i) (wr_dbg_paths[i]++)
#else
#define WR_DBG_PATH(i) ((void)0)
#endif
#if defined(WRHIP_TIMING) && !defined(WRHIP_HOSTSIM)
__device__ unsigned long long wr_dbg_tp[16384 * 8];
#define WR_TP(i) do { __builtin_amdgcn_s_waitcnt(0); const int g_ = (int)(blockIdx.x * blockDim.x + threadIdx.x); if (g_ < 16384) wr_dbg_tp[g_ * 8 + (i)] = wall_clock64(); } while (0)
#else
#define WR_TP(i) ((void)0)
#endif
struct wf2 { float x, y; };
struct wf4 { float x, y, z, w; };
struct wi4 { int x, y, z, w; };

WR_DEVICE float wr_min(float a, float b) { return a < b ? a : b; }
WR_DEVICE float wr_max(float a, float b) { return a > b ? a : b; }
WR_DEVICE float wr_clamp(float a, float lo, float hi) { return wr_min(wr_max(a, lo), hi); }
// ... 2404 lines not shown
    float xl = wr_accum(S.lx, S.ls, ya - S.lrow), xr = wr_accum(S.rx, S.rs, ya - S.rrow);
    float lu = 0.0f, lv = 0.0f, ru = 0.0f, rv = 0.0f, wl = 0.0f, wr = 0.0f, zl = 0.0f, zr = 0.0f;
    if (stride >= 6) {
      lu = wr_accum(S.luv[0], S.luvs[0], ya - S.lrow); lv = wr_accum(S.luv[1], S.luvs[1], ya - S.lrow);
      ru = wr_accum(S.ruv[0], S.ruvs[0], ya - S.rrow); rv = wr_accum(S.ruv[1], S.ruvs[1], ya - S.rrow);
    }
    if (stride >= 10) {
      wl = wr_accum(Q.persp.lw[i], Q.persp.lws[i], ya - S.lrow); wr = wr_accum(Q.persp.rw[i], Q.persp.rws[i], ya - S.rrow);
      zl = wr_accum(Q.persp.lz[i], Q.persp.lzs[i], ya - S.lrow); zr = wr_accum(Q.persp.rz[i], Q.persp.rzs[i], ya - S.rrow);
    }
    const float ls = S.ls, rs = S.rs, lus = S.luvs[0], lvs = S.luvs[1], rus = S.ruvs[0], rvs = S.ruvs[1];
    const float lws = stride >= 10 ? Q.persp.lws[i] : 0.0f, rws = stride >= 10 ? Q.persp.rws[i] : 0.0f;
    const float lzs = stride >= 10 ? Q.persp.lzs[i] : 0.0f, rzs = stride >= 10 ? Q.persp.rzs[i] : 0.0f;
    float* __restrict__ e = tab + (size_t)(ya - P.y0) * (size_t)stride;
    if (stride == 2) {
      int y = ya;
      if (((y - P.y0) & 1) && y < yb) { e[0] = xl; e[1] = xr; xl = xl + ls; xr = xr + rs; y++; e += 2; }
      for (; y + 2 <= yb; y += 2, e += 4) {
        const float xl1 = xl + ls, xr1 = xr + rs;
        wr_store16(e, xl, xr, xl1, xr1);
        xl = xl1 + ls; xr = xr1 + rs;
      }
      if (y < yb) { e[0] = xl; e[1] = xr; }
    } else {
      for (int y = ya; y < yb; y++, e += stride) {
        e[0] = xl; e[1] = xr; e[2] = lu; e[3] = lv; e[4] = ru; e[5] = rv;
        xl = xl + ls; xr = xr + rs; lu = lu + lus; lv = lv + lvs; ru = ru + rus; rv = rv + rvs;
        if (stride >= 10) {
          e[6] = wl; e[7] = wr; e[8] = zl; e[9] = zr;
          wl = wl + lws; wr = wr + rws; zl = zl + lzs; zr = zr + rzs;
        }
      }
      if (stride >= 14) {
        float l2u = wr_accum(Q.persp.l2u[i], Q.persp.l2us[i], ya - S.lrow), l2v = wr_accum(Q.persp.l2v[i], Q.persp.l2vs[i], ya - S.lrow);
        float r2u = wr_accum(Q.persp.r2u[i], Q.persp.r2us[i], ya - S.rrow), r2v = wr_accum(Q.persp.r2v[i], Q.persp.r2vs[i], ya - S.rrow);
        const float l2us = Q.persp.l2us[i], l2vs = Q.persp.l2vs[i], r2us = Q.persp.r2us[i], r2vs = Q.persp.r2vs[i];
        float* __restrict__ e2 = tab + (size_t)(ya - P.y0) * (size_t)stride;
        for (int y = ya; y < yb; y++, e2 += stride) {
          e2[10] = l2u; e2[11] = l2v; e2[12] = r2u; e2[13] = r2v;
          l2u = l2u + l2us; l2v = l2v + l2vs; r2u = r2u + r2us; r2v = r2v + r2vs;
        }
      }
    }
  }
  Q.rowtab_y0 = P.y0; Q.rowtab_rows = rows; Q.rowtab_stride = stride;
  Q.rowtab = tab;
#ifdef WRHIP_HOSTSIM
  { static const bool dbg = getenv("WRHIP_DEBUG_QTAB") != nullptr; if (dbg) fprintf(stderr, "row table: kind %d rows %d stride %d at word %lld of %u\n", (int)P.kind, rows, stride, (long long)(tab - T.qtab), T.qtab_cap); }
#endif
}
WR_DEVICE bool wr_quad_row_span(const WrQuadRec& Q, int y, int& s0, int& s1) {
  int si = -1;
  for (int i = 0; i < Q.nseg; i++) if (y >= Q.seg[i].row_a && y < Q.seg[i].row_b) si = i;
  if (si < 0) return false;
  const WrQuadSeg& S = Q.seg[si];
  float xl, xr;
  wr_quad_row_x(Q, S, y, xl, xr);
  if (!Q.aa) {
    s0 = int(floorf(wr_clamp(xl, S.b0, S.b1) + 0.5f)); s1 = int(floorf(wr_clamp(xr, S.b0, S.b1) + 0.5f));
  } else {
    const float radl = 0.5f * fabsf(S.ls), radr = 0.5f * fabsf(S.rs);
    s0 = S.lmask ? int(floorf(wr_clamp(xl - radl, S.b0, S.b1))) : int(floorf(wr_clamp(xl, S.b0, S.b1) + 0.5f));
    s1 = S.rmask ? int(ceilf(wr_clamp(xr + radr, S.b0, S.b1))) : int(floorf(wr_clamp(xr, S.b0, S.b1) + 0.5f));
  }
  return true;
}

static_assert(offsetof(WrQuadRec, yuv) >= sizeof(WrYuvRec), "the YUV record moves into the quad record's union: the two must not overlap");
WR_DEVICE bool wr_yuv_persp_ok(const WrVsOut& o, const WrYuvRec& Y) {
  if (Y.format != 3) return true;
  bool same = true;
  for (int n = 0; n < 4; n++) {
    uint32_t a, b, c, e;
    __builtin_memcpy(&a, &o.u2[n], 4); __builtin_memcpy(&b, &o.u3[n], 4); __builtin_memcpy(&c, &o.v2[n], 4); __builtin_memcpy(&e, &o.v3[n], 4);
    same = same && a == b && c == e;
  }
  return same;
}
WR_DEVICE void wr_copy_words(void* dst, const void* src, int bytes) {
  int32_t* d = (int32_t*)dst; const int32_t* s = (const int32_t*)src;
  for (int i = 0; i < bytes / 4; i++) d[i] = s[i];
}

WR_DEVICE void wr_finish_prim(const WrDrawDesc& d, int draw_index, const WrVsOut& o, WrPrim& P, WrAux* auxp,
                              WrUnsupportedCounters* cnt) {
  P.kind = WR_PK_NONE;
  P.draw = draw_index;
  P.color[0] = P.color[1] = 0; P.z = 0; P.tex_slot = 0;
  P.uv_add[0] = o.uv_add[0]; P.uv_add[1] = o.uv_add[1];
  P.dual = o.dual; P.dual_swz = o.dual_swz;
  P.blend = (int16_t)d.blend;
  P.flags = d.flags & (WR_PF_DEPTH_TEST | WR_PF_DEPTH_WRITE | WR_PF_DEPTH_LESS);
  P.x0 = P.y0 = P.x1 = P.y1 = 0;
  const bool persp = o.pw[1] != o.pw[0] || o.pw[2] != o.pw[0] || o.pw[3] != o.pw[0];
  float w = 1.0f / o.pw[0];
  if (!wr_isfinite(w)) w = 0.0f;
  float sx[4], sy[4], pz3[4], pw3[4];
  bool clipped = false;
  if (persp) {
    bool inside = true;
    for (int n = 0; n < 4; n++) inside = inside && (o.pz[n] > -o.pw[n]) && (o.pz[n] < o.pw[n]);
    const bool ptex = ((d.shader == WR_SH_PS_QUAD_TEXTURED || o.persp_div >= 0.0f) && (o.kind == WR_PK_TEX_RGBA8 || o.kind == WR_PK_TEX_FS)) ||
                      ((d.shader == WR_SH_PS_TEXT_RUN || d.shader == WR_SH_PS_TEXT_RUN_DUAL) && (o.kind == WR_PK_TEX_R8 || o.kind == WR_PK_TEX_RGBA8)) ||
                      o.kind == WR_PK_FILTER || o.kind == WR_PK_MIX_BLEND || (o.kind == WR_PK_QUAD_MASK && auxp->clip.w == 1.0f) ||
                      (o.kind == WR_PK_YUV && inside && wr_yuv_persp_ok(o, auxp->yuv)) || (o.kind == WR_PK_TEX_REPEAT && o.persp_div >= 0.0f) || (o.kind == WR_PK_GRADIENT && (d.shader == WR_SH_BRUSH_LINEAR_GRADIENT || d.shader == WR_SH_BRUSH_LINEAR_GRADIENT_ALPHA ||
                                                                              d.shader == WR_SH_PS_QUAD_RADIAL_GRADIENT || d.shader == WR_SH_PS_QUAD_CONIC_GRADIENT));
    if (!(o.kind == WR_PK_SOLID || ptex)) { atomicAdd(&cnt->perspective_prims, 1u); return; }
    clipped = !inside;
    if (clipped) {
      WrClipStash& St = *wr_clip_stash(auxp->quad);
      for (int n = 0; n < 4; n++) { St.px[n] = o.px[n]; St.py[n] = o.py[n]; St.pz[n] = o.pz[n]; St.pw[n] = o.pw[n]; St.u[n] = o.u[n]; St.v[n] = o.v[n]; }
      St.two = o.kind == WR_PK_MIX_BLEND ? 1 : 0;
      if (St.two) for (int n = 0; n < 4; n++) { St.u2[n] = o.u2[n]; St.v2[n] = o.v2[n]; }
    }
    const float scx = d.vp_size[0] * 0.5f, scy = d.vp_size[1] * 0.5f;
    const float ofx = d.vp_origin[0] + scx, ofy = d.vp_origin[1] + scy;
    for (int n = 0; n < 4; n++) {
      const float wn = clipped ? 0.0f : 1.0f / o.pw[n];
      sx[n] = o.px[n] * wn * scx + ofx;
      sy[n] = o.py[n] * wn * scy + ofy;
      pz3[n] = o.pz[n] * wn * 0.5f + 0.5f;
      pw3[n] = wn;
    }
  } else {
    for (int n = 0; n < 4; n++) {
      sx[n] = (o.px[n] * w + 1.0f) * 0.5f * d.vp_size[0] + d.vp_origin[0];
      sy[n] = (o.py[n] * w + 1.0f) * 0.5f * d.vp_size[1] + d.vp_origin[1];
      pz3[n] = 0.f; pw3[n] = 0.f;
    }
  }
  float cx0 = float(d.clip[0]), cy0 = float(d.clip[1]), cx1 = float(d.clip[2]), cy1 = float(d.clip[3]);
  bool masked = false;
  if (o.has_mask && d.blend != WR_BLEND_NONE) {
    const WrTexDesc& mt = d.tex[WR_S_CLIP_MASK];
    if (mt.format != WR_FMT_R8 || !mt.ptr || o.kind == WR_PK_BLUR || o.kind == WR_PK_CLIP_RECT || o.kind == WR_PK_BOX_SHADOW) {
      P.kind = WR_PK_UNSUPPORTED; atomicAdd(&cnt->unsupported_prims, 1u); return;
    }
    int bx0 = int(o.mask_bb[0]), by0 = int(o.mask_bb[1]);
    int bx1 = bx0 + int(o.mask_bb[2]), by1 = by0 + int(o.mask_bb[3]);
    bx0 = wr_imax(bx0, 0); by0 = wr_imax(by0, 0); bx1 = wr_imin(bx1, mt.width); by1 = wr_imin(by1, mt.height);
    const int offx = int(o.mask_offset[0]) + int(d.vp_origin[0]), offy = int(o.mask_offset[1]) + int(d.vp_origin[1]);
    cx0 = wr_max(cx0, float(bx0 + offx)); cy0 = wr_max(cy0, float(by0 + offy));
    cx1 = wr_min(cx1, float(bx1 + offx)); cy1 = wr_min(cy1, float(by1 + offy));
    P.mask_off[0] = offx; P.mask_off[1] = offy;
    masked = true;
  }
#ifdef WRHIP_HOSTSIM
  if (getenv("WRHIP_DEBUG_VS"))
    fprintf(stderr, "    vs: pos (%g %g %g %g) (%g %g) (%g %g) (%g %g) screen (%g %g) (%g %g) (%g %g) (%g %g)\n", o.px[0], o.py[0], o.pz[0],
            o.pw[0], o.px[1], o.py[1], o.px[2], o.py[2], o.px[3], o.py[3], sx[0], sy[0], sx[1], sy[1], sx[2], sy[2], sx[3], sy[3]);
#endif
  int sides = 0;
  for (int n = 0; n < 4; n++) {
    sides |= sx[n] < cx1 ? (sx[n] > cx0 ? 3 : 1) : 2;
    sides |= sy[n] < cy1 ? (sy[n] > cy0 ? 12 : 4) : 8;
  }
  if (sides != 0xF && !clipped) return;
  if (!persp) {
    float screenZ = (o.pz[0] * w + 1.0f) * 0.5f;
    if (screenZ < 0.0f || screenZ > 1.0f) return;
    P.z = uint32_t(16777215.0f * screenZ);
  }

  const bool aa = o.aa_edges != 0 && d.blend != WR_BLEND_NONE;
  if (o.dual && ((o.aa_edges != 0 && d.blend != WR_BLEND_NONE) || persp) && o.kind != WR_PK_TEX_REPEAT) { P.kind = WR_PK_UNSUPPORTED; atomicAdd(&cnt->unsupported_prims, 1u); return; }
  const bool texq = (d.flags & WR_DF_QUADS) &&
                    (o.kind == WR_PK_TEX_RGBA8 || o.kind == WR_PK_TEX_FS || o.kind == WR_PK_TEX_R8 || o.kind == WR_PK_TEX_REPEAT ||
                     o.kind == WR_PK_GRADIENT || o.kind == WR_PK_FILTER || o.kind == WR_PK_QUAD_MASK || (o.kind == WR_PK_SOLID && masked) ||
                     o.kind == WR_PK_MIX_BLEND || o.kind == WR_PK_YUV);
  if (aa && (o.kind != WR_PK_SOLID || masked) && !texq) {
    P.kind = WR_PK_UNSUPPORTED; atomicAdd(&cnt->unsupported_prims, 1u); return;
  }
  bool typeA = sy[0] == sy[1] && sy[2] == sy[3] && sx[0] == sx[3] && sx[1] == sx[2];
  bool typeB = sx[0] == sx[1] && sx[2] == sx[3] && sy[0] == sy[3] && sy[1] == sy[2];
  if ((!typeA && !typeB) || (aa && texq) || persp) {
    const bool solidq = o.kind == WR_PK_SOLID && !masked && !(d.flags & WR_DF_SIMPLE);
    if (persp && !solidq && !(texq && (o.kind == WR_PK_TEX_RGBA8 || o.kind == WR_PK_TEX_FS || o.kind == WR_PK_TEX_R8 || o.kind == WR_PK_TEX_REPEAT || o.kind == WR_PK_FILTER || o.kind == WR_PK_GRADIENT || o.kind == WR_PK_QUAD_MASK || (o.kind == WR_PK_SOLID && masked) || o.kind == WR_PK_MIX_BLEND || o.kind == WR_PK_YUV))) {
      atomicAdd(&cnt->perspective_prims, 1u); return;
    }
    if (!solidq && !texq) {
      P.kind = WR_PK_UNSUPPORTED; atomicAdd(&cnt->unsupported_prims, 1u); return;
    }
    union { WrRepeatRec rep; WrGradRec grad; WrFilterRec filt; WrClipRec clip; WrMixRec mix; } base;
    if (o.kind == WR_PK_MIX_BLEND) base.mix = auxp->mix;
    if (o.kind == WR_PK_TEX_REPEAT) base.rep = auxp->rep;
    else if (o.kind == WR_PK_GRADIENT) base.grad = auxp->grad;
    else if (o.kind == WR_PK_FILTER) base.filt = auxp->filt;
    else if (o.kind == WR_PK_QUAD_MASK) base.clip = auxp->clip;
    if (o.kind == WR_PK_YUV && !clipped) wr_copy_words(&auxp->quad.yuv, &auxp->yuv, sizeof(WrYuvRec));
    int bx0, by0, bx1, by1;
    float qu[4], qv[4];
    for (int n = 0; n < 4; n++) { qu[n] = persp ? o.u[n] * pw3[n] : o.u[n]; qv[n] = persp ? o.v[n] * pw3[n] : o.v[n]; }
    if (clipped) {
      WrClipStash& St = *wr_clip_stash(auxp->quad);
      St.cx0 = cx0; St.cy0 = cy0; St.cx1 = cx1; St.cy1 = cy1; St.aa = aa ? 1 : 0; St.aa_edges = o.aa_edges;
      St.vp[0] = d.vp_origin[0]; St.vp[1] = d.vp_origin[1]; St.vp[2] = d.vp_size[0]; St.vp[3] = d.vp_size[1];
      auxp->quad.nseg = -1; auxp->quad.rowtab = nullptr; auxp->quad.rowtab_rows = 0;
      bx0 = int(cx0); by0 = int(cy0); bx1 = int(cx0) + 1; by1 = int(cy0) + 1;
    }
    else if ((o.kind == WR_PK_MIX_BLEND && persp) || o.kind == WR_PK_YUV) {
      float qu2[4], qv2[4], z4[4], w4[4];
      for (int n = 0; n < 4; n++) {
        qu2[n] = persp ? o.u2[n] * pw3[n] : o.u2[n]; qv2[n] = persp ? o.v2[n] * pw3[n] : o.v2[n];
        z4[n] = persp ? pz3[n] : o.u3[n]; w4[n] = persp ? pw3[n] : o.v3[n];
      }
      if (!wr_quad_walk(sx, sy, qu, qv, cx0, cy0, cx1, cy1, aa, o.aa_edges, auxp->quad, bx0, by0, bx1, by1, z4, w4, true, qu2, qv2)) return;
    }
    else if (o.kind == WR_PK_MIX_BLEND) {
      if (!wr_quad_walk(sx, sy, qu, qv, cx0, cy0, cx1, cy1, aa, o.aa_edges, auxp->quad, bx0, by0, bx1, by1, o.u2, o.v2, true)) return;
    }
    else if (!wr_quad_walk(sx, sy, qu, qv, cx0, cy0, cx1, cy1, aa, o.aa_edges, auxp->quad, bx0, by0, bx1, by1, pz3, pw3, persp)) return;
    auxp->quad.pad = persp ? ((o.kind == WR_PK_SOLID && d.shader != WR_SH_PS_QUAD_TEXTURED) ? 1 : 2) : 0;
    if (persp) auxp->quad.persp.div = o.persp_div;
    P.x0 = wr_imax(bx0, int(cx0)); P.x1 = wr_imin(bx1, int(cx1)); P.y0 = wr_imax(by0, int(cy0)); P.y1 = wr_imin(by1, int(ceilf(cy1)));
    if (o.cd[2] >= o.cd[0]) { P.x0 = wr_imax(P.x0, o.cd[0]); P.y0 = wr_imax(P.y0, o.cd[1]); P.x1 = wr_imin(P.x1, o.cd[2]); P.y1 = wr_imin(P.y1, o.cd[3]); }
    if (P.x1 <= P.x0 || P.y1 <= P.y0) return;
    P.rows_linear = 0;
    if (solidq) {
      P.kind = WR_PK_SOLID_QUAD;
      wr_pack_color(o.color, P.color);
      return;
    }
    P.kind = WR_PK_TEX_QUAD;
    auxp->quad.base_kind = o.kind == WR_PK_SOLID ? (int)WR_PK_SOLID_MASKED : o.kind;
    if (o.kind == WR_PK_SOLID) wr_pack_color(o.color, P.color);
    if (o.kind == WR_PK_TEX_REPEAT) auxp->quad.rep = base.rep;
    else if (o.kind == WR_PK_GRADIENT) auxp->quad.grad = base.grad;
    else if (o.kind == WR_PK_FILTER) auxp->quad.filt = base.filt;
    else if (o.kind == WR_PK_QUAD_MASK) auxp->quad.clip = base.clip;
    else if (o.kind == WR_PK_MIX_BLEND) auxp->quad.mix = base.mix;
    if (masked) P.flags |= WR_PF_MASKED;
    if (o.has_color) { P.flags |= WR_PF_HAS_COLOR; wr_pack_color(o.color, P.color); }
    if (o.tail_clamp) P.flags |= WR_PF_TAIL_CLAMP;
    if (o.tail_modulate) P.flags |= WR_PF_TAIL_MODULATE;
    P.tex_slot = o.tex_slot;
    P.uv_bounds[0] = o.uv_bounds.x; P.uv_bounds[1] = o.uv_bounds.y; P.uv_bounds[2] = o.uv_bounds.z; P.uv_bounds[3] = o.uv_bounds.w;
    P.fcolor[0] = o.color.x; P.fcolor[1] = o.color.y; P.fcolor[2] = o.color.z; P.fcolor[3] = o.color.w;
    if (o.blend_override != 0 && d.blend != WR_BLEND_NONE) { P.blend = (int16_t)o.blend_override; wr_pack_color(o.blend_color, P.color); }
    return;
  }
  float xa = sx[0], xb = sx[2], ya = sy[0], yb = sy[2];
  float xmin = wr_min(xa, xb), xmax = wr_max(xa, xb), ymin = wr_min(ya, yb), ymax = wr_max(ya, yb);
  float sx0 = wr_clamp(xmin, cx0, cx1), sx1 = wr_clamp(xmax, cx0, cx1);
  int ix0 = int(floorf(sx0 + 0.5f)), ix1 = int(floorf(sx1 + 0.5f));
  float aaRound = 0.5f;
  if (aa) {
    int li, ri;
    if (typeA) { const bool flipx = sx[0] > sx[1]; li = flipx ? 2 : 0; ri = flipx ? 0 : 2; }
    else { const bool flipx = sx[0] > sx[3]; li = flipx ? 3 : 1; ri = flipx ? 1 : 3; }
    const bool ml = (o.aa_edges >> li) & 1, mr = (o.aa_edges >> ri) & 1;
    const int l_start = ml ? int(floorf(sx0)) : int(floorf(sx0 + 0.5f));
    const int l_end = ml ? int(ceilf(sx0)) : int(floorf(sx0 + 0.5f));
    const int r_end = mr ? int(ceilf(sx1)) : int(floorf(sx1 + 0.5f));
    ix0 = l_start; ix1 = r_end;
    WrAARec& A = auxp->aa;
    const float dxl = (-1.0f * 256.0f) * (1.0f / sqrtf(1.0f + 0.0f * 0.0f)), dxr = (1.0f * 256.0f) * (1.0f / sqrtf(1.0f + 0.0f * 0.0f));
    A.lstart = ml ? 128.0f + dxl * (xmin - 0.5f) : 256.0f; A.lend = ml ? -dxl : 0.0f;
    A.rstart = mr ? 128.0f + dxr * (xmax - 0.5f) : 256.0f; A.rend = mr ? -dxr : 0.0f;
    A.laa_end = l_end;
    aaRound = 0.0f;
  }
  float ystart = floorf(wr_max(wr_min(ymin, cy1), cy0) + aaRound) + 0.5f;
  float ylimit = wr_min(ymax, cy1);
  int iy0 = int(ystart);
  int iy1 = int(floorf(ylimit - 0.5f)) + 1;
  while ((float(iy1) + 0.5f) <= ylimit) iy1++;
  while (iy1 > iy0 && (float(iy1 - 1) + 0.5f) > ylimit) iy1--;
  if (o.cd[2] >= o.cd[0]) { ix0 = wr_imax(ix0, o.cd[0]); ix1 = wr_imin(ix1, o.cd[2]); iy1 = wr_imin(iy1, o.cd[3]); }
  if (ix1 <= ix0 || iy1 <= iy0) return;
  P.x0 = ix0; P.x1 = ix1; P.y0 = iy0; P.y1 = iy1;
  P.kind = (masked && o.kind == WR_PK_SOLID) ? (int16_t)WR_PK_SOLID_MASKED : (aa ? (int16_t)WR_PK_SOLID_AA : (int16_t)o.kind);
  if (masked && o.kind != WR_PK_SOLID) P.flags |= WR_PF_MASKED;
  P.rows_linear = 0;
  if ((d.flags & WR_DF_SIMPLE) && P.kind != WR_PK_SOLID) {
    P.kind = WR_PK_UNSUPPORTED; atomicAdd(&cnt->unsupported_prims, 1u); return;
  }
  if (o.kind == WR_PK_UNSUPPORTED) { atomicAdd(&cnt->unsupported_prims, 1u); return; }
  const bool blend_override = o.blend_override != 0 && d.blend != WR_BLEND_NONE;
  if (o.kind == WR_PK_SOLID) {
    wr_pack_color(o.color, P.color);
    if (masked) P.tex_slot = WR_S_CLIP_MASK;
  } else if (o.kind == WR_PK_TEX_RGBA8 || o.kind == WR_PK_TEX_R8 || o.kind == WR_PK_BLUR || o.kind == WR_PK_TEX_FS || o.kind == WR_PK_CLIP_RECT || o.kind == WR_PK_BOX_SHADOW || o.kind == WR_PK_GRADIENT || o.kind == WR_PK_FILTER || o.kind == WR_PK_MIX_BLEND || o.kind == WR_PK_SVG_FILTER || o.kind == WR_PK_YUV || o.kind == WR_PK_QUAD_MASK || o.kind == WR_PK_TEX_REPEAT || o.kind == WR_PK_BORDER_SOLID || o.kind == WR_PK_BORDER_SEGMENT || o.kind == WR_PK_FAST_GRADIENT || o.kind == WR_PK_LINE_DECORATION) {
    if (o.has_color) { P.flags |= WR_PF_HAS_COLOR; wr_pack_color(o.color, P.color); }
    if (o.tail_clamp) P.flags |= WR_PF_TAIL_CLAMP;
    if (o.tail_modulate) P.flags |= WR_PF_TAIL_MODULATE;
    P.tex_slot = o.tex_slot;
    P.uv_bounds[0] = o.uv_bounds.x; P.uv_bounds[1] = o.uv_bounds.y;
    P.uv_bounds[2] = o.uv_bounds.z; P.uv_bounds[3] = o.uv_bounds.w;
    P.fcolor[0] = o.color.x; P.fcolor[1] = o.color.y; P.fcolor[2] = o.color.z; P.fcolor[3] = o.color.w;
    int tl = 0, tr = 0, bl = 0, br = 0;
    for (int n = 0; n < 4; n++) {
      bool left = sx[n] == xmin, top = sy[n] == ymin;
      if (left && top) tl = n; else if (!left && top) tr = n; else if (left) bl = n; else br = n;
    }
    float yScale = 1.0f / wr_max(ymax - ymin, 1.0f / 256.0f);
    float dy0 = ystart - ymin;
    float lsu = (wr_pick4(o.u, bl) - wr_pick4(o.u, tl)) * yScale, lsv = (wr_pick4(o.v, bl) - wr_pick4(o.v, tl)) * yScale;
    float rsu = (wr_pick4(o.u, br) - wr_pick4(o.u, tr)) * yScale, rsv = (wr_pick4(o.v, br) - wr_pick4(o.v, tr)) * yScale;
    P.uvL0[0] = wr_pick4(o.u, tl) + dy0 * lsu; P.uvL0[1] = wr_pick4(o.v, tl) + dy0 * lsv;
    P.uvR0[0] = wr_pick4(o.u, tr) + dy0 * rsu; P.uvR0[1] = wr_pick4(o.v, tr) + dy0 * rsv;
    P.uvLs[0] = lsu; P.uvLs[1] = lsv; P.uvRs[0] = rsu; P.uvRs[1] = rsv;
    P.xl = xmin; P.xr = xmax;
    {
      const int rows = iy1 - iy0 - 1;
      P.rows_linear = (wr_accum_is_linear(P.uvL0[0], lsu, rows) && wr_accum_is_linear(P.uvL0[1], lsv, rows) &&
                       wr_accum_is_linear(P.uvR0[0], rsu, rows) && wr_accum_is_linear(P.uvR0[1], rsv, rows)) ? 1 : 0;
    }
    if (o.kind == WR_PK_MIX_BLEND) {
      WrMixRec& M = auxp->mix;
      const float l2u = (wr_pick4(o.u2, bl) - wr_pick4(o.u2, tl)) * yScale, l2v = (wr_pick4(o.v2, bl) - wr_pick4(o.v2, tl)) * yScale;
      const float r2u = (wr_pick4(o.u2, br) - wr_pick4(o.u2, tr)) * yScale, r2v = (wr_pick4(o.v2, br) - wr_pick4(o.v2, tr)) * yScale;
      M.sL0[0] = wr_pick4(o.u2, tl) + dy0 * l2u; M.sL0[1] = wr_pick4(o.v2, tl) + dy0 * l2v;
      M.sR0[0] = wr_pick4(o.u2, tr) + dy0 * r2u; M.sR0[1] = wr_pick4(o.v2, tr) + dy0 * r2v;
      M.sLs[0] = l2u; M.sLs[1] = l2v; M.sRs[0] = r2u; M.sRs[1] = r2v;
    }
    if (o.kind == WR_PK_SVG_FILTER) {
      WrSvgRec& M = auxp->svg;
      const float l2u = (wr_pick4(o.u2, bl) - wr_pick4(o.u2, tl)) * yScale, l2v = (wr_pick4(o.v2, bl) - wr_pick4(o.v2, tl)) * yScale;
      const float r2u = (wr_pick4(o.u2, br) - wr_pick4(o.u2, tr)) * yScale, r2v = (wr_pick4(o.v2, br) - wr_pick4(o.v2, tr)) * yScale;
      M.sL0[0] = wr_pick4(o.u2, tl) + dy0 * l2u; M.sL0[1] = wr_pick4(o.v2, tl) + dy0 * l2v;
      M.sR0[0] = wr_pick4(o.u2, tr) + dy0 * r2u; M.sR0[1] = wr_pick4(o.v2, tr) + dy0 * r2v;
      M.sLs[0] = l2u; M.sLs[1] = l2v; M.sRs[0] = r2u; M.sRs[1] = r2v;
    }
    if (o.kind == WR_PK_YUV) {
      WrYuvRec& Y = auxp->yuv;
      for (int pl = 1; pl < 3; pl++) {
        const float* pu = pl == 1 ? o.u2 : o.u3; const float* pv = pl == 1 ? o.v2 : o.v3;
        const float u4[4] = {pu[0], pu[1], pu[2], pu[3]}, v4[4] = {pv[0], pv[1], pv[2], pv[3]};
        const float l2u = (wr_pick4(u4, bl) - wr_pick4(u4, tl)) * yScale, l2v = (wr_pick4(v4, bl) - wr_pick4(v4, tl)) * yScale;
        const float r2u = (wr_pick4(u4, br) - wr_pick4(u4, tr)) * yScale, r2v = (wr_pick4(v4, br) - wr_pick4(v4, tr)) * yScale;
        float* L0 = pl == 1 ? Y.uL0 : Y.vL0; float* Ls = pl == 1 ? Y.uLs : Y.vLs; float* R0 = pl == 1 ? Y.uR0 : Y.vR0; float* Rs = pl == 1 ? Y.uRs : Y.vRs;
        L0[0] = wr_pick4(u4, tl) + dy0 * l2u; L0[1] = wr_pick4(v4, tl) + dy0 * l2v;
        R0[0] = wr_pick4(u4, tr) + dy0 * r2u; R0[1] = wr_pick4(v4, tr) + dy0 * r2v;
        Ls[0] = l2u; Ls[1] = l2v; Rs[0] = r2u; Rs[1] = r2v;
      }
    }
    if (o.kind == WR_PK_BOX_SHADOW) {
      WrBoxRec& B = auxp->box;
      const float l2u = (wr_pick4(o.u2, bl) - wr_pick4(o.u2, tl)) * yScale, l2v = (wr_pick4(o.v2, bl) - wr_pick4(o.v2, tl)) * yScale;
      const float r2u = (wr_pick4(o.u2, br) - wr_pick4(o.u2, tr)) * yScale, r2v = (wr_pick4(o.v2, br) - wr_pick4(o.v2, tr)) * yScale;
      B.lpL0[0] = wr_pick4(o.u2, tl) + dy0 * l2u; B.lpL0[1] = wr_pick4(o.v2, tl) + dy0 * l2v;
      B.lpR0[0] = wr_pick4(o.u2, tr) + dy0 * r2u; B.lpR0[1] = wr_pick4(o.v2, tr) + dy0 * r2v;
      B.lpLs[0] = l2u; B.lpLs[1] = l2v; B.lpRs[0] = r2u; B.lpRs[1] = r2v;
    }
  }
  if (blend_override) {
    P.blend = (int16_t)o.blend_override;
    wr_pack_color(o.blend_color, P.color);
  }
}


struct WrWide { uint32_t bg, ra; };

WR_DEVICE WrWide wr_unpack(uint32_t p) {
  WrWide w;
  w.bg = (p & 0xFF) | ((p & 0xFF00) << 8);
  w.ra = ((p >> 16) & 0xFF) | ((p >> 24) << 16);
  return w;
}
WR_DEVICE uint32_t wr_pack1(uint32_t v) {
  uint32_t m = v > 255u ? 0xFFFFu : 0u;
// ... 976 lines not shown
  const float start = float(P.x0) + 0.5f - P.xl;
  t.ou = Lu + t.su * start;
  const int len = P.x1 - P.x0;
  t.span = len >= 4 ? (len & ~3) : 0;
  const float q0x = t.ou * W * qs + qo, q1x = (t.ou + t.su) * W * qs + qo;
  t.stepx = 4.0f * (q1x - q0x);
  t.minx = wr_max(P.uv_bounds[0] * W * qs + qo, 0.0f);
  t.maxx = wr_max(P.uv_bounds[2] * W * qs + qo, t.minx);
  t.miny = wr_max(P.uv_bounds[1] * H * qs + qo, 0.0f);
  t.maxy = wr_max(P.uv_bounds[3] * H * qs + qo, t.miny);
  t.ub0 = P.uv_bounds[0]; t.ub1 = P.uv_bounds[1]; t.ub2 = P.uv_bounds[2]; t.ub3 = P.uv_bounds[3];
  t.lv0 = P.uvL0[1]; t.lvs = P.uvLs[1]; t.y0 = P.y0;
  const int need = WR_PF_TAIL_CLAMP | WR_PF_TAIL_MODULATE | WR_PF_HAS_COLOR;
  t.simple = (tex.ptr && P.uvLs[0] == 0.0f && P.uvRs[0] == 0.0f && P.uvL0[1] == P.uvR0[1] && P.uvLs[1] == P.uvRs[1] &&
              (P.flags & need) == need && !(P.flags & WR_PF_MASKED) && ((P.color[0] | P.color[1]) & 0xFF00FF00u) == 0 && tex.width >= 2) ? 1 : 0;
  t.fcolor[0] = P.fcolor[0]; t.fcolor[1] = P.fcolor[1]; t.fcolor[2] = P.fcolor[2]; t.fcolor[3] = P.fcolor[3];
  t.unit = 0; t.ix0 = t.iy0 = 0; t.tix[0] = t.tix[1] = t.tix[2] = 0;
  const int rows = P.y1 - P.y0;
  if (t.simple && len <= 128 && rows <= 128) {
    bool ok = true;
    int q0 = 0;
    for (int n = 0; n < len && ok; n++) {
      const bool tail = n >= t.span;
      const int lane = (tail ? n - t.span : n) & 3;
      float lu = t.ou;
      for (int i = 0; i < lane; i++) lu += t.su;
      int qx;
      if (!tail) {
        qx = int(wr_clamp(wr_accum(lu * W * qs + qo, t.stepx, n >> 2), t.minx, t.maxx));
        if (n == 0) q0 = qx;
        ok = qx == q0 + 128 * n;
      } else {
        if (t.span > 0) lu = lu + (t.su * 4.0f) * (float(t.span) * 0.25f);
        qx = int(wr_clamp(lu, t.ub0, t.ub2) * W * 128.0f + (0.5f - 64.0f));
        const int k = n - t.span;
        if (k == 0) t.tix[0] = qx >> 7; else if (k == 1) t.tix[1] = qx >> 7; else t.tix[2] = qx >> 7;
      }
      ok = ok && (qx & 0x7F) == 0 && qx >= 0 && (qx >> 7) <= tex.width - 2;
    }
    int r0 = 0;
    float ov = t.lv0;
    for (int r = 0; r < rows && ok; r++, ov += t.lvs) {
      const int qs_ = int(wr_clamp(ov * H * qs + qo, t.miny, t.maxy));
      const int qt_ = int(wr_clamp(ov, t.ub1, t.ub3) * H * 128.0f + (0.5f - 64.0f));
      if (r == 0) r0 = qs_;
      ok = qs_ == r0 + 128 * r && qt_ == qs_ && (qs_ & 0x7F) == 0 && qs_ >= 0 && (qs_ >> 7) <= tex.height - 1;
    }
    if (ok && rows > 0) { t.unit = 1; t.ix0 = q0 >> 7; t.iy0 = r0 >> 7; }
  }
  return t;
}

WR_DEVICE void wr_write_glyph_rec(const WrTargetDesc& T, int gid, const WrPrim& P, const WrTexRec& t) {
  if (!T.grecs) return;
  WrGlyphRec g;
  g.x0 = (int16_t)P.x0; g.y0 = (int16_t)P.y0; g.x1 = (int16_t)P.x1; g.y1 = (int16_t)P.y1;
  g.c0 = P.color[0]; g.c1 = P.color[1];
  g.stride = t.stride;
  const int len = P.x1 - P.x0;
  const int ix0 = t.span > 0 ? t.ix0 : t.tix[0];
  g.base = (uint64_t)(unsigned long long)t.ptr + (uint64_t)((long long)(t.iy0 - t.y0) * (long long)t.stride + (long long)(ix0 - P.x0));
  const int tail_x = t.span >= len ? P.x1 : P.x0 + t.span;
  const long long th = (long long)(t.wh >> 16), last = (long long)(t.iy0 + (P.y1 - P.y0) - 1) * (long long)t.stride + (long long)ix0 + 3;
  bool ok = t.simple != 0 && t.unit != 0 && len >= 1 && (len >= 4 || last < th * (long long)t.stride) && (P.blend == WR_BLEND_NONE || P.blend == WR_BLEND_PREMULT) &&
            P.x0 >= -32768 && P.y0 >= -32768 && P.x1 <= 32767 && P.y1 <= 32767;
  for (int k = 0; k < 3; k++)
    if (tail_x + k < P.x1) ok = ok && (k == 0 ? t.tix[0] : (k == 1 ? t.tix[1] : t.tix[2])) == ix0 + (tail_x - P.x0) + k;
  g.fcolor[0] = t.fcolor[0]; g.fcolor[1] = t.fcolor[1]; g.fcolor[2] = t.fcolor[2]; g.fcolor[3] = t.fcolor[3];
  g.info = ok ? (1u | ((P.flags & WR_PF_DEPTH_TEST) ? 2u : 0u) | (uint32_t(P.blend & 0xFF) << 8) | (uint32_t(uint16_t(int16_t(tail_x))) << 16)) : 0u;
  ((WrGlyphRec*)T.grecs)[gid] = g;
#ifdef WRHIP_HOSTSIM
  if (getenv("WRHIP_DEBUG_GLYPHS")) {
    static int n_ok = 0, n_bad = 0, n_nounit = 0, n_narrow = 0;
    if (ok) n_ok++; else { n_bad++; if (!t.unit || !t.simple) n_nounit++; if (len < 4) n_narrow++; }
    if (((n_ok + n_bad) & 1023) == 0 || getenv("WRHIP_DEBUG_GLYPHS")[0] == '2') fprintf(stderr, "glyph recs: %d eligible, %d not (%d not unit / simple, %d narrower than 4)\n", n_ok, n_bad, n_nounit, n_narrow);
  }
#endif
}

#ifdef WRHIP_TIMING
__device__ unsigned long long wr_dbg_mid[16384];
__device__ unsigned wr_dbg_prim[16384 * 4];
#endif
WR_DEVICE void wr_vertex_prim(const WrDescView& V, int n_draws, const uint8_t* __restrict__ arena,
                              int gid, WrPrim& P, WrAux* aux, WrUnsupportedCounters* cnt) {
  P.blend = 0; P.flags = 0; P.z = 0; P.color[0] = P.color[1] = 0; P.tex_slot = 0;
  P.uv_add[0] = P.uv_add[1] = 0.0f; P.rows_linear = 0; P.dual = 0; P.dual_swz = 0.0f;
  P.uv_add[0] = P.uv_add[1] = 0.0f; P.rows_linear = 0; P.dual = 0; P.dual_swz = 0.0f;
  int lo = V.lo0;
  while (lo + 1 < n_draws && V.draw(lo + 1).first_prim <= gid) lo++;
  const WrDrawDesc& d = V.draw(lo);
  int inst = gid - d.first_prim;
  WR_TP(2);
  if (inst >= d.count) {
    P.kind = WR_PK_NONE; P.x0 = P.x1 = P.y0 = P.y1 = 0; P.draw = lo;
    return;
  }
  if (d.shader == WR_SH_CLEAR_OP) {
    P.kind = WR_PK_CLEAR; P.blend = WR_BLEND_NONE; P.draw = lo; P.z = d.clear_depth;
    P.flags = d.flags & (WR_PF_CLEAR_COLOR | WR_PF_CLEAR_DEPTH);
    P.x0 = d.clip[0]; P.y0 = d.clip[1]; P.x1 = d.clip[2]; P.y1 = d.clip[3];
    P.color[0] = d.clear_color; P.color[1] = 0;
    if (P.x1 <= P.x0 || P.y1 <= P.y0) P.kind = WR_PK_NONE;
    return;
  }
  WrVsOut o;
  o.tex_slot = 0; o.uv_bounds = wf4{0, 0, 0, 0}; o.tail_clamp = 0; o.tail_modulate = 0;
  o.uv_add[0] = o.uv_add[1] = 0.0f;
  o.blend_override = 0; o.blend_color = wf4{0, 0, 0, 0}; o.persp_div = -1.0f; o.dual = 0; o.dual_swz = 0.0f;
  o.cd[0] = o.cd[1] = 0; o.cd[2] = o.cd[3] = -1;
  switch (d.shader) {
    case WR_SH_PS_QUAD_TEXTURED: wr_vs_ps_quad_textured(d, arena, inst, o); break;
    case WR_SH_PS_QUAD_MASK: wr_vs_ps_quad_textured(d, arena, inst, o, 1, &aux[gid].clip); break;
    case WR_SH_PS_QUAD_MASK_FAST: wr_vs_ps_quad_textured(d, arena, inst, o, 2, &aux[gid].clip); break;
    case WR_SH_PS_QUAD_RADIAL_GRADIENT: wr_vs_ps_quad_textured(d, arena, inst, o, 3, nullptr, &aux[gid].grad); break;
    case WR_SH_PS_QUAD_CONIC_GRADIENT: wr_vs_ps_quad_textured(d, arena, inst, o, 4, nullptr, &aux[gid].grad); break;
    case WR_SH_BRUSH_SOLID:
    case WR_SH_BRUSH_SOLID_ALPHA: wr_vs_brush(d, arena, inst, 0, o); break;
    case WR_SH_BRUSH_IMAGE: wr_vs_brush(d, arena, inst, 1, o); break;
    case WR_SH_BRUSH_IMAGE_ALPHA: wr_vs_brush(d, arena, inst, 2, o); break;
    case WR_SH_BRUSH_IMAGE_DUAL: wr_vs_brush(d, arena, inst, 9, o); break;
    case WR_SH_BRUSH_OPACITY:
    case WR_SH_BRUSH_OPACITY_ALPHA: wr_vs_brush(d, arena, inst, 7, o); break;
    case WR_SH_BRUSH_IMAGE_REPEAT: wr_vs_brush(d, arena, inst, 5, o, nullptr, nullptr, &aux[gid].rep); break;
    case WR_SH_BRUSH_IMAGE_REPEAT_ALPHA: wr_vs_brush(d, arena, inst, 6, o, nullptr, nullptr, &aux[gid].rep); break;
    case WR_SH_BRUSH_IMAGE_REPEAT_DUAL: wr_vs_brush(d, arena, inst, 11, o, nullptr, nullptr, &aux[gid].rep); break;
    case WR_SH_BRUSH_LINEAR_GRADIENT:
    case WR_SH_BRUSH_LINEAR_GRADIENT_ALPHA: wr_vs_brush(d, arena, inst, 3, o, &aux[gid].grad); break;
    case WR_SH_BRUSH_BLEND:
    case WR_SH_BRUSH_BLEND_ALPHA: wr_vs_brush(d, arena, inst, 4, o, nullptr, &aux[gid].filt); break;
    case WR_SH_BRUSH_MIX_BLEND:
    case WR_SH_BRUSH_MIX_BLEND_ALPHA: wr_vs_brush(d, arena, inst, 8, o, nullptr, nullptr, nullptr, &aux[gid].mix); break;
    case WR_SH_BRUSH_YUV:
    case WR_SH_BRUSH_YUV_ALPHA: wr_vs_brush(d, arena, inst, 10, o, nullptr, nullptr, nullptr, nullptr, &aux[gid].yuv); break;
    case WR_SH_COMPOSITE_YUV: wr_vs_composite_yuv(d, arena, inst, o, aux[gid].yuv); break;
    case WR_SH_COMPOSITE: wr_vs_composite(d, arena, inst, false, o); break;
    case WR_SH_COMPOSITE_FAST: wr_vs_composite(d, arena, inst, true, o); break;
    case WR_SH_PS_CLEAR: wr_vs_ps_clear(d, arena, inst, o); break;
    case WR_SH_PS_TEXT_RUN: wr_vs_ps_text_run(d, arena, inst, false, o); break;
    case WR_SH_PS_TEXT_RUN_DUAL: wr_vs_ps_text_run(d, arena, inst, true, o); break;
    case WR_SH_PS_TEXT_RUN_GT: wr_vs_ps_text_run(d, arena, inst, false, o, true); break;
    case WR_SH_PS_TEXT_RUN_DUAL_GT: wr_vs_ps_text_run(d, arena, inst, true, o, true); break;
    case WR_SH_CS_BLUR_ALPHA: wr_vs_cs_blur(d, arena, inst, o, aux[gid].blur); break;
    case WR_SH_CS_BLUR_COLOR: wr_vs_cs_blur(d, arena, inst, o, aux[gid].blur); break;
    case WR_SH_CS_CLIP_RECT: wr_vs_cs_clip_rect(d, arena, inst, false, o, aux[gid].clip); break;
    case WR_SH_CS_CLIP_RECT_FAST: wr_vs_cs_clip_rect(d, arena, inst, true, o, aux[gid].clip); break;
    case WR_SH_CS_CLIP_BOX_SHADOW: wr_vs_cs_clip_box_shadow(d, arena, inst, o, aux[gid].box); break;
    case WR_SH_CS_SCALE: wr_vs_cs_scale(d, arena, inst, V.target(d.target).format, o); break;
    case WR_SH_PS_COPY: wr_vs_ps_copy(d, arena, inst, o); break;
    case WR_SH_CS_SVG_FILTER: wr_vs_cs_svg_filter(d, arena, inst, false, o, aux[gid].svg); break;
    case WR_SH_CS_SVG_FILTER_NODE: wr_vs_cs_svg_filter(d, arena, inst, true, o, aux[gid].svg); break;
    case WR_SH_PS_SPLIT_COMPOSITE: wr_vs_ps_split_composite(d, arena, inst, o); break;
    case WR_SH_CS_BORDER_SOLID: wr_vs_cs_border_solid(d, arena, inst, o, aux[gid].border); break;
    case WR_SH_CS_BORDER_SEGMENT: wr_vs_cs_border_segment(d, arena, inst, o, aux[gid].bseg); break;
    case WR_SH_CS_FAST_LINEAR_GRADIENT: wr_vs_cs_fast_linear_gradient(d, arena, inst, o, aux[gid].fgrad); break;
    case WR_SH_CS_LINE_DECORATION: wr_vs_cs_line_decoration(d, arena, inst, o, aux[gid].line); break;
    case WR_SH_CS_LINEAR_GRADIENT: wr_vs_cs_linear_gradient(d, arena, inst, o, &aux[gid].grad); break;
    case WR_SH_CS_RADIAL_GRADIENT: wr_vs_cs_radial_gradient(d, arena, inst, o, &aux[gid].grad); break;
    case WR_SH_CS_CONIC_GRADIENT: wr_vs_cs_conic_gradient(d, arena, inst, o, &aux[gid].grad); break;
    default:
      P.kind = WR_PK_NONE; P.x0 = P.x1 = P.y0 = P.y1 = 0; P.draw = lo; P.blend = 0; P.flags = 0; P.z = 0;
      P.color[0] = P.color[1] = 0;
      return;
  }
#ifdef WRHIP_TIMING
  if (gid < 16384) wr_dbg_mid[gid] = wall_clock64();
#endif
  WR_TP(6);
  wr_finish_prim(d, lo, o, P, &aux[gid], cnt);
  if ((P.kind == WR_PK_SOLID_QUAD || P.kind == WR_PK_TEX_QUAD) && aux[gid].quad.nseg < 0) {
    int bx0, by0, bx1, by1;
    float cx0, cy0, cx1, cy1;
    bool ok = wr_persp_clipped_walk(aux[gid].quad, bx0, by0, bx1, by1, cx0, cy0, cx1, cy1);
    if (ok) {
      P.x0 = wr_imax(bx0, int(cx0)); P.x1 = wr_imin(bx1, int(cx1)); P.y0 = wr_imax(by0, int(cy0)); P.y1 = wr_imin(by1, int(ceilf(cy1)));
      ok = P.x1 > P.x0 && P.y1 > P.y0;
    }
    if (!ok) { P.kind = WR_PK_NONE; P.x0 = P.x1 = P.y0 = P.y1 = 0; aux[gid].quad.nseg = 0; }
  }
  if (P.kind == WR_PK_SOLID_QUAD || P.kind == WR_PK_TEX_QUAD) wr_quad_build_rowtab(&V.target(d.target), &P, &aux[gid].quad);
  if ((P.kind == WR_PK_SOLID_QUAD || P.kind == WR_PK_TEX_QUAD) && aux[gid].quad.pad != 0 && (P.flags & WR_PF_DEPTH_TEST)) {
    uint32_t* fr = V.target(d.target).flat_rows;
    if (fr) {
      bool any = false;
      for (int y = P.y0; y < P.y1; y++) {
        int s0, s1;
        if (wr_quad_row_span(aux[gid].quad, y, s0, s1) && wr_imin(s1, P.x1) > wr_imax(s0, P.x0)) { atomicMin(&fr[y], (uint32_t)gid); any = true; }
      }
      if (any) atomicMin(&fr[V.target(d.target).height], (uint32_t)gid);
    }
  }
  if (d.query_slot >= 0 && P.kind != WR_PK_NONE && P.kind != WR_PK_UNSUPPORTED) {
    unsigned long long n = 0;
    if (P.kind == WR_PK_SOLID_QUAD || P.kind == WR_PK_TEX_QUAD) {
      for (int y = P.y0; y < P.y1; y++) { int s0, s1; if (wr_quad_row_span(aux[gid].quad, y, s0, s1)) { s0 = wr_imax(s0, P.x0); s1 = wr_imin(s1, P.x1); if (s1 > s0) n += (unsigned long long)(s1 - s0); } }
    } else {
      n = (unsigned long long)(P.x1 - P.x0) * (unsigned long long)(P.y1 - P.y0);
    }
    if (n) atomicAdd(&cnt->samples[d.query_slot & (WR_QUERY_SLOTS - 1)], n);
  }
}


WR_DEVICE void wr_bin_prim(const WrPrim& P, bool valid, int gid, const WrDescView& V, unsigned long long* masks) {
  const WrTargetDesc* targets = V.targets;
  int bx0 = 0, bx1 = -1, by0 = 0, by1 = -1, tgt = -1, rel = 0;
  if (valid && P.kind != WR_PK_NONE && P.kind != WR_PK_UNSUPPORTED) {
    tgt = V.draw(P.draw).target;
    const WrTargetDesc& T = V.target(tgt);
    bx0 = wr_imax(P.x0, 0) / WR_BIN_W; bx1 = (wr_imin(P.x1, T.width) - 1) / WR_BIN_W;
    by0 = wr_imax(P.y0, 0) / WR_BIN_H; by1 = (wr_imin(P.y1, T.height) - 1) / WR_BIN_H;
    by0 = wr_imax(by0, T.y_begin / WR_BIN_H); by1 = wr_imin(by1, (T.y_end - 1) / WR_BIN_H);
    rel = gid - T.first_prim;
    if (T.rows_mode) bx1 = -1;
  }
  const bool has = tgt >= 0 && bx1 >= bx0 && by1 >= by0;
#ifdef WRHIP_HOSTSIM
  if (has) {
    const WrTargetDesc& T = targets[tgt];
    unsigned long long* base = masks + (size_t)T.word_base + (rel >> 6);
    for (int by = by0; by <= by1; by++)
      for (int bx = bx0; bx <= bx1; bx++) atomicOr(&base[(size_t)(by * T.bins_x + bx) * T.words_per_bin], 1ull << (rel & 63));
  }
#else
  typedef short wr_s2 __attribute__((ext_vector_type(2)));
  const int lane = threadIdx.x & 63;
  unsigned long long todo = __ballot(has);
  while (todo) {
    const int leader = __builtin_ctzll(todo);
    const int s_tgt = __builtin_amdgcn_readlane(tgt, leader), s_word = __builtin_amdgcn_readlane(rel >> 6, leader);
    const bool mine = has && tgt == s_tgt && (rel >> 6) == s_word;
    todo &= ~__ballot(mine);
    const int s_shift = __builtin_amdgcn_readlane((rel & 63) - lane, leader);
    const WrTargetDesc& T = V.target(s_tgt);
    const int bins_x = T.bins_x, wpb = T.words_per_bin;
    unsigned long long* base = masks + (size_t)T.word_base + s_word;
    wr_s2 lo2 = {(short)(mine ? bx0 : 32767), (short)(mine ? by0 : 32767)};
    wr_s2 hi2 = {(short)(mine ? bx1 : -1), (short)(mine ? by1 : -1)};
#pragma unroll
    for (int d = 1; d < 64; d <<= 1) {
      const wr_s2 ol = __builtin_bit_cast(wr_s2, __shfl_xor(__builtin_bit_cast(int, lo2), d));
      const wr_s2 oh = __builtin_bit_cast(wr_s2, __shfl_xor(__builtin_bit_cast(int, hi2), d));
      lo2 = __builtin_elementwise_min(lo2, ol); hi2 = __builtin_elementwise_max(hi2, oh);
    }
    const int ux0 = __builtin_amdgcn_readfirstlane((int)lo2.x), uy0 = __builtin_amdgcn_readfirstlane((int)lo2.y);
    const int ux1 = __builtin_amdgcn_readfirstlane((int)hi2.x), uy1 = __builtin_amdgcn_readfirstlane((int)hi2.y);
    for (int cx0 = ux0; cx0 <= ux1; cx0 += 64) {
      const int W = wr_imin(64, ux1 - cx0 + 1);
      unsigned xlo = 0, xhi = 0;
      for (int i = 0; i < W; i++) {
        const unsigned long long m = __ballot(mine && bx0 <= cx0 + i && bx1 >= cx0 + i);
        xlo = lane == i ? (unsigned)m : xlo;
        xhi = lane == i ? (unsigned)(m >> 32) : xhi;
      }
      const float rW = 1.0f / float(W);
      for (int ry0 = uy0; ry0 <= uy1; ry0 += 64) {
        const int H = wr_imin(64, uy1 - ry0 + 1);
        unsigned ylo = 0, yhi = 0;
        for (int j = 0; j < H; j++) {
          const unsigned long long m = __ballot(mine && by0 <= ry0 + j && by1 >= ry0 + j);
          ylo = lane == j ? (unsigned)m : ylo;
          yhi = lane == j ? (unsigned)(m >> 32) : yhi;
        }
        for (int idx = lane; idx < W * H + lane; idx += 64) {
          const bool live = idx < W * H;
          const int row = live ? int((float(idx) + 0.5f) * rW) : 0;
          const int col = live ? idx - row * W : 0;
          const unsigned wlo = (unsigned)__shfl((int)xlo, col) & (unsigned)__shfl((int)ylo, row);
          const unsigned whi = (unsigned)__shfl((int)xhi, col) & (unsigned)__shfl((int)yhi, row);
          unsigned long long w = ((unsigned long long)whi << 32) | wlo;
          w = s_shift >= 0 ? (w << s_shift) : (w >> -s_shift);
          if (live && w) atomicOr(&base[(size_t)((ry0 + row) * bins_x + cx0 + col) * wpb], w);
        }
      }
    }
  }
#endif
// ... 179 lines not shown
  return br;
}

WR_DEVICE float wr_box_map_v(const WrBoxRec& B, float vl) {
  float v = wr_clamp(vl, 0.0f, B.edge[1]);
  v += wr_max(0.0f, vl - B.edge[3]);
  return (B.uv_noclamp[3] - B.uv_noclamp[1]) * v + B.uv_noclamp[1];
}
WR_DEVICE WrBoxKey wr_box_row_key(const WrPrim& P, const WrBoxRec& B, const WrRowVals& r, const WrBoxRow& b) {
  WrBoxKey k;
  k.valid = (r.s[1] == 0.0f && r.s[3] == 0.0f && B.w > 0.0f) ? 1 : 0;
  k.o0 = r.o[0]; k.s0 = r.s[0]; k.o2 = r.o[2]; k.s2 = r.s[2];
  k.ss_se = b.ss_se; k.os01 = b.os01; k.os23 = b.os23;
  const float w = 1.0f / B.w;
  k.mv_mul = wr_box_map_v(B, r.o[1] * w); k.mv_div = wr_box_map_v(B, r.o[1] / B.w);
  const float l = r.o[3] * w, ld = r.o[3] / B.w;
  k.in_mul = wr_step01(B.bounds[1], l) - wr_step01(B.bounds[3], l);
  k.in_div = wr_step01(B.bounds[1], ld) - wr_step01(B.bounds[3], ld);
  return k;
}
WR_DEVICE bool wr_box_keys_equal(const WrBoxKey& a, const WrBoxKey& b) {
  return a.valid && b.valid && a.o0 == b.o0 && a.s0 == b.s0 && a.o2 == b.o2 && a.s2 == b.s2 && a.ss_se == b.ss_se && a.os01 == b.os01 &&
         a.os23 == b.os23 && a.mv_mul == b.mv_mul && a.mv_div == b.mv_div && a.in_mul == b.in_mul && a.in_div == b.in_div;
}

WR_DEVICE void wr_mask_rows_take(const WrTargetDesc& T, unsigned long long ns, unsigned long long nr, unsigned long long nb, uint32_t pitch,
                                 uint32_t tabs16, int gid, int target, WrRec* __restrict__ recs, int& slot_out) {
  WrMaskSlot sl;
  sl.prim = gid; sl.target = target; sl.row0 = uint32_t(nr); sl.pitch = pitch; sl.off16 = uint32_t(nb);
  sl.pad[0] = 1u; sl.pad[1] = tabs16; sl.pad[2] = 0;
  sl.key.valid = 0;
  T.mr_slots[ns] = sl;
  slot_out = int(ns);
  const unsigned long long addr = (unsigned long long)(T.mr_store + nb * 16);
  recs[gid].kbf = (recs[gid].kbf & ~0xFFu) | WR_PK_MASK_ROWS;
  recs[gid].c0 = uint32_t(addr); recs[gid].c1 = uint32_t(addr >> 32); recs[gid].z = pitch;
}
WR_DEVICE bool wr_mask_rows_cas(const WrTargetDesc& T, unsigned long long slots, unsigned long long rows, unsigned long long n16, unsigned long long& base) {
  unsigned long long old = *(volatile unsigned long long*)T.mr_ctl;
  for (;;) {
    const unsigned long long ns = old >> 48, nr = (old >> 28) & 0xFFFFFull, nb = old & 0xFFFFFFFull;
    if (ns + slots > T.mr_max_slots || nr + rows > WR_MR_MAX_ROWS || nb + n16 > T.mr_cap16) return false;
    const unsigned long long want = ((ns + slots) << 48) | ((nr + rows) << 28) | (nb + n16);
    const unsigned long long seen = atomicCAS(T.mr_ctl, old, want);
    if (seen == old) { base = old; return true; }
    old = seen;
  }
}
WR_DEVICE void wr_mask_rows_reserve(const WrTargetDesc* T, uint32_t rows, uint32_t pitch, unsigned long long n16, uint32_t tabs16,
                                    int gid, int target, WrRec* __restrict__ recs, int& slot_out) {
  slot_out = -1;
#ifndef WRHIP_HOSTSIM
  const int lane = threadIdx.x & 63;
  const unsigned long long m = __ballot(T != nullptr);
  if (!m) return;
  uint32_t pre_slots = 0, pre_rows = 0, tot_slots = 0, tot_rows = 0;
  unsigned long long pre_n16 = 0, tot_n16 = 0;
  for (unsigned long long mm = m; mm; mm &= mm - 1ull) {
    const int i = __builtin_ctzll(mm);
    const uint32_t ri = (uint32_t)__builtin_amdgcn_readlane((int)rows, i);
    const unsigned long long ni = (unsigned long long)(uint32_t)__builtin_amdgcn_readlane((int)(uint32_t)n16, i) |
                                  ((unsigned long long)(uint32_t)__builtin_amdgcn_readlane((int)(uint32_t)(n16 >> 32), i) << 32);
    if (lane == i) { pre_slots = tot_slots; pre_rows = tot_rows; pre_n16 = tot_n16; }
    tot_slots += 1u; tot_rows += ri; tot_n16 += ni;
  }
  const int lead = __builtin_ctzll(m);
  unsigned long long base = 0ull;
  int ok = 0;
  if (lane == lead) ok = wr_mask_rows_cas(*T, tot_slots, tot_rows, tot_n16, base) ? 1 : 0;
  ok = __builtin_amdgcn_readlane(ok, lead);
  if (ok) {
    const unsigned long long b = (unsigned long long)(uint32_t)__builtin_amdgcn_readlane((int)(uint32_t)base, lead) |
                                 ((unsigned long long)(uint32_t)__builtin_amdgcn_readlane((int)(uint32_t)(base >> 32), lead) << 32);
    if (T) wr_mask_rows_take(*T, (b >> 48) + pre_slots, ((b >> 28) & 0xFFFFFull) + pre_rows, (b & 0xFFFFFFFull) + pre_n16, pitch, tabs16, gid, target, recs, slot_out);
    return;
  }
#endif
  if (T) {
    unsigned long long base;
    if (wr_mask_rows_cas(*T, 1, rows, n16, base)) wr_mask_rows_take(*T, base >> 48, (base >> 28) & 0xFFFFFull, base & 0xFFFFFFFull, pitch, tabs16, gid, target, recs, slot_out);
  }
}

WR_DEVICE void wr_setup_body(const WrDrawDesc* __restrict__ draws, int n_draws,
                                const uint8_t* __restrict__ arena, WrPrim* __restrict__ prims,
                                WrRec* __restrict__ recs, WrAux* __restrict__ aux, int n_prims,
                                const WrTargetDesc* __restrict__ targets, unsigned long long* __restrict__ masks,
                                float* __restrict__ vtab, WrUnsupportedCounters* cnt, const int* __restrict__ blk, const int bid) {
  const int gid = bid * (int)blockDim.x + (int)threadIdx.x;
  const bool valid = gid < n_prims;
  WrPrim P;
  P.kind = WR_PK_NONE; P.draw = 0; P.x0 = P.y0 = P.x1 = P.y1 = 0;
#ifdef WRHIP_TIMING
  const int dbg_mode = n_draws >> 24;
  n_draws &= 0xFFFFFF;
  if (dbg_mode == 1) return;
  const unsigned long long tm0 = wall_clock64();
#endif
  WR_TP(0);
  WrDescView V;
  V.draws = draws; V.targets = targets; V.ld = nullptr; V.lt = nullptr; V.lo0 = 0; V.nk = 0; V.t0 = V.t1 = -1;
  {
    const int nblk = (n_prims + 63) >> 6;
    const int b = wr_imin(gid >> 6, nblk - 1);
#if defined(WRHIP_HOSTSIM) || !defined(WR_DESC_STAGE)
    V.lo0 = ((const WrBlock*)blk)[b].lo0;
#else
    __shared__ __attribute__((aligned(16))) unsigned long long wr_sd_lds[4 * WR_SD_WAVE_Q];
    const wr_u4 bw = wr_load16((const void*)((const WrBlock*)blk + b));
    V.lo0 = __builtin_amdgcn_readfirstlane((int)bw.x);
    const int wave = (int)threadIdx.x >> 6, lane = (int)threadIdx.x & 63;
    if (blockDim.x <= 256u) {
      V.nk = __builtin_amdgcn_readfirstlane((int)bw.y); V.t0 = __builtin_amdgcn_readfirstlane((int)bw.z); V.t1 = __builtin_amdgcn_readfirstlane((int)bw.w);
      unsigned long long* L = wr_sd_lds + wave * WR_SD_WAVE_Q;
      const unsigned long long* gd = (const unsigned long long*)(draws + V.lo0);
      const unsigned long long* g0 = (const unsigned long long*)(targets + wr_imax(V.t0, 0));
      const unsigned long long* g1 = (const unsigned long long*)(targets + wr_imax(V.t1, 0));
      for (int i = lane; i < V.nk * WR_SD_DRAW_Q; i += 64) L[i] = gd[i];
      if (V.nk > 0) for (int i = lane; i < WR_SD_TGT_Q; i += 64) L[2 * WR_SD_DRAW_Q + i] = g0[i];
      if (V.nk > 1) for (int i = lane; i < WR_SD_TGT_Q; i += 64) L[2 * WR_SD_DRAW_Q + WR_SD_TGT_Q + i] = g1[i];
      __builtin_amdgcn_fence(__ATOMIC_RELEASE, "workgroup"); __builtin_amdgcn_wave_barrier(); __builtin_amdgcn_fence(__ATOMIC_ACQUIRE, "workgroup");
      V.ld = (const WrDrawDesc*)L; V.lt = (const WrTargetDesc*)(L + 2 * WR_SD_DRAW_Q);
    }
#endif
  }
  WR_TP(1);
  if (valid) wr_vertex_prim(V, n_draws, arena, gid, P, aux, cnt);
  WR_TP(7);
#ifdef WRHIP_TIMING
  const unsigned long long tm1 = wall_clock64();
  if (dbg_mode == 2) { if (valid && P.x0 == 12345678) prims[gid] = P; return; }
#endif
  const WrTargetDesc* mr_T = nullptr;
  uint32_t mr_rows = 0, mr_pitch = 0;
  unsigned long long mr_n16 = 0;
  uint32_t mr_tabs16 = 0;
  if (valid) {
    const WrDrawDesc& D_ = V.draw(P.draw);
    const WrTargetDesc& T_ = V.target(D_.target);
    const WrRec rec_ = wr_make_rec(P, T_.format);
    recs[gid] = rec_;
    if (T_.rows_mode || ((rec_.kbf & 0xFF) != WR_PK_SOLID_FOLDED && (rec_.kbf & 0xFF) != WR_PK_NONE)) prims[gid] = P;
    if ((P.kind == WR_PK_BOX_SHADOW || P.kind == WR_PK_CLIP_RECT) && (D_.flags & WR_DF_MASK_ROWS) && P.x1 > P.x0 && P.y1 > P.y0) {
      const WrTargetDesc& T = T_;
      if (T.mr_ctl) {
        mr_T = &T;
        mr_rows = uint32_t(P.y1 - P.y0); mr_pitch = uint32_t(((P.x1 + 3) & ~3) - (P.x0 & ~3));
        const unsigned long long map16 = ((unsigned long long)mr_rows * 4 + 15) >> 4;
        mr_n16 = map16 + (((unsigned long long)mr_rows * mr_pitch + 15) >> 4);
        mr_tabs16 = uint32_t(mr_n16);
        mr_n16 += WR_ACCTABS_N16;
      }
    }
    if (P.kind == WR_PK_TEX_R8) {
      aux[gid].tex = wr_make_texrec(P, D_.tex[P.tex_slot]);
      wr_write_glyph_rec(T_, gid, P, aux[gid].tex);
    }
    if (P.kind == WR_PK_SOLID_MASKED) {
      const WrTexDesc& mt = D_.tex[WR_S_CLIP_MASK];
      WrTexRec t;
      __builtin_memset(&t, 0, sizeof(t));
      t.ptr = mt.ptr; t.stride = mt.stride; t.wh = uint32_t(mt.width) | (uint32_t(mt.height) << 16);
      t.span = 0x40000000; t.y0 = P.y0;
      t.simple = ((P.color[0] | P.color[1]) & 0xFF00FF00u) == 0 ? 1 : 0;
      t.unit = 1; t.ix0 = P.x0 - P.mask_off[0]; t.iy0 = P.y0 - P.mask_off[1];
      aux[gid].tex = t;
      wr_write_glyph_rec(T_, gid, P, t);
    }
    if (P.kind == WR_PK_TEX_RGBA8) {
      const WrDrawDesc& d = D_;
      WrTexRec T;
      const int rows = P.y1 - P.y0;
      if (wr_texrow_x_setup(P, d.tex[P.tex_slot], T, cnt) && (T.simple == 3 || (d.vtab_base >= 0 && rows <= d.vtab_rows))) {
        if (T.simple == 2) {
          T.iy0 = d.vtab_base + (gid - d.first_prim) * d.vtab_rows;
          float* vp = vtab + T.iy0;
          const float st = T.lvs;
          float v = T.lv0;
          int k = 0;
          for (; k + 4 <= rows; k += 4) {
            const float a = v, b = a + st, c = b + st, e = c + st;
            v = e + st;
            vp[k] = a; vp[k + 1] = b; vp[k + 2] = c; vp[k + 3] = e;
          }
          for (; k < rows; k++, v += st) vp[k] = v;
        }
        aux[gid].tex = T;
      } else {
        aux[gid].tex.simple = 0;
      }
    }
  }
  int mr_slot = -1;
  wr_mask_rows_reserve(mr_T, mr_rows, mr_pitch, mr_n16, mr_tabs16, gid, V.draw(P.draw).target, recs, mr_slot);
  if (mr_slot >= 0) {
    WrMaskSlot& sl = mr_T->mr_slots[mr_slot];
    WrAccTabs* tabs = (WrAccTabs*)(mr_T->mr_store + ((size_t)sl.off16 + mr_tabs16) * 16);
    const bool box = P.kind == WR_PK_BOX_SHADOW;
    const WrBoxRec& B = aux[gid].box;
    const float s0[8] = {P.uvL0[0], P.uvL0[1], P.uvR0[0], P.uvR0[1], box ? B.lpL0[0] : 0.0f, box ? B.lpL0[1] : 0.0f, box ? B.lpR0[0] : 0.0f, box ? B.lpR0[1] : 0.0f};
    const float st[8] = {P.uvLs[0], P.uvLs[1], P.uvRs[0], P.uvRs[1], box ? B.lpLs[0] : 0.0f, box ? B.lpLs[1] : 0.0f, box ? B.lpRs[0] : 0.0f, box ? B.lpRs[1] : 0.0f};
    wr_acctabs_build(tabs, box ? 8 : 4, s0, st, int(mr_rows) - 1, P.rows_linear != 0);
    if (box) {
      const int yc = P.y0 + (int(mr_rows) >> 1);
      const WrRowVals rvc = wr_box_row_vals(P, B, yc, tabs);
      sl.key = wr_box_row_key(P, B, rvc, wr_box_row_setup(P, B, rvc));
    }
  }
  {
    WrGradRec* Gq = nullptr;
    if (valid && P.kind == WR_PK_GRADIENT) Gq = &aux[gid].grad;
    else if (valid && P.kind == WR_PK_TEX_QUAD && aux[gid].quad.base_kind == WR_PK_GRADIENT) Gq = &aux[gid].quad.grad;
    wr_grad_tables_wave(V, P.draw, gid, Gq);
    if (Gq) wr_grad_merge_bits(Gq);
  }
#ifdef WRHIP_TIMING
  const unsigned long long tm2 = wall_clock64();
  if (valid && gid < 16384) { wr_dbg_prim[gid * 4] = (unsigned)(tm1 - tm0); wr_dbg_prim[gid * 4 + 1] = (unsigned)(tm2 - tm1); wr_dbg_prim[gid * 4 + 2] = (unsigned)(wr_dbg_mid[gid] - tm0); wr_dbg_prim[gid * 4 + 3] = (unsigned)draws[P.draw].shader; }
#endif
#ifdef WRHIP_TIMING
  if (dbg_mode == 3) return;
#endif
  wr_bin_prim(P, valid, gid, V, masks);
#ifdef WRHIP_TIMING
  const unsigned long long tm3 = wall_clock64();
  if ((threadIdx.x & 63) == 0) {
    atomicAdd(&cnt->dbg[0], (unsigned)(tm1 - tm0)); atomicAdd(&cnt->dbg[1], (unsigned)(tm2 - tm1)); atomicAdd(&cnt->dbg[2], (unsigned)(tm3 - tm2));
    atomicAdd(&cnt->dbg[3], 1u);
    if (bid == (n_prims - 1) / (int)blockDim.x) atomicAdd(&cnt->dbg[4], (unsigned)(tm3 - tm0));
    atomicMax(&cnt->dbg[5], (unsigned)(tm3 - tm0));
  }
#endif
}

#ifndef WR_INST_ONLY
__global__ void __launch_bounds__(256, 3) wr_setup_kernel(const WrDrawDesc* __restrict__ draws, int n_draws,
                                const uint8_t* __restrict__ arena, WrPrim* __restrict__ prims,
                                WrRec* __restrict__ recs, WrAux* __restrict__ aux, int n_prims,
                                const WrTargetDesc* __restrict__ targets, unsigned long long* __restrict__ masks,
                                float* __restrict__ vtab, WrUnsupportedCounters* cnt, const int* __restrict__ blk) {
  wr_setup_body(draws, n_draws, arena, prims, recs, aux, n_prims, targets, masks, vtab, cnt, blk, (int)blockIdx.x);
}
#endif
```

webrender_amd/glapi.py:

```python
import ctypes as C
import os

c_void_p, c_char_p = C.c_void_p, C.c_char_p
i32, u32, u8, f32, f64 = C.c_int32, C.c_uint32, C.c_uint8, C.c_float, C.c_double
u64, isz, usz = C.c_uint64, C.c_ssize_t, C.c_size_t
P = c_void_p

SIGNATURES = {
    "ActiveTexture": (None, [u32]),
    "BindTexture": (None, [u32, u32]),
    "BindBuffer": (None, [u32, u32]),
    "BindVertexArray": (None, [u32]),
    "BindFramebuffer": (None, [u32, u32]),
    "BindRenderbuffer": (None, [u32, u32]),
    "BlendFunc": (None, [u32, u32, u32, u32]),
    "BlendColor": (None, [f32, f32, f32, f32]),
    "BlendEquation": (None, [u32]),
    "Enable": (None, [u32]),
    "Disable": (None, [u32]),
    "GenQueries": (None, [i32, P]),
    "BeginQuery": (None, [u32, u32]),
    "EndQuery": (None, [u32]),
    "GetQueryObjectui64v": (None, [u32, u32, P]),
    "GenBuffers": (None, [i32, P]),
# ... 24 lines not shown
    "Uniform1i": (None, [i32, i32]),
    "Uniform4fv": (None, [i32, i32, P]),
    "UniformMatrix4fv": (None, [i32, i32, u8, P]),
    "DrawElementsInstanced": (None, [u32, i32, u32, isz, i32]),
    "EnableVertexAttribArray": (None, [u32]),
    "VertexAttribDivisor": (None, [u32, u32]),
    "LinkProgram": (None, [u32]),
    "GetLinkStatus": (i32, [u32]),
    "UseProgram": (None, [u32]),
    "SetViewport": (None, [i32, i32, i32, i32]),
    "FramebufferRenderbuffer": (None, [u32, u32, u32, u32]),
    "RenderbufferStorage": (None, [u32, u32, i32, i32]),
    "DepthMask": (None, [u8]),
    "DepthFunc": (None, [u32]),
    "SetScissor": (None, [i32, i32, i32, i32]),
    "ClearColor": (None, [f32, f32, f32, f32]),
    "ClearDepth": (None, [f64]),
    "Clear": (None, [u32]),
    "ClearTexSubImage": (None, [u32, i32, i32, i32, i32, i32, i32, i32, u32, u32, P]),
    "ClearTexImage": (None, [u32, i32, u32, u32, P]),
    "ClearColorRect": (None, [u32, i32, i32, i32, i32, f32, f32, f32, f32]),
    "PixelStorei": (None, [u32, i32]),
    "ReadPixels": (None, [i32, i32, i32, i32, u32, u32, P]),
    "Finish": (None, []),
    "ShaderSourceByName": (None, [u32, c_char_p]),
    "TexParameteri": (None, [u32, u32, i32]),
    "CopyImageSubData": (None, [u32, u32, i32, i32, i32, i32, u32, u32, i32, i32, i32, i32, i32, i32, i32]),
    "CopyTexSubImage2D": (None, [u32, i32, i32, i32, i32, i32, i32, i32]),
    "BlitFramebuffer": (None, [i32, i32, i32, i32, i32, i32, i32, i32, u32, u32]),
    "GetIntegerv": (None, [u32, P]),
    "GetBooleanv": (None, [u32, P]),
    "GetString": (c_char_p, [u32]),
    "GetStringi": (c_char_p, [u32, u32]),
    "GetError": (u32, []),
    "InitDefaultFramebuffer": (None, [i32, i32, i32, i32, i32, P]),
    "GetColorBuffer": (P, [u32, u8, P, P, P]),
    "ResolveFramebuffer": (None, [u32]),
    "SetTextureBuffer": (None, [u32, u32, i32, i32, i32, P, i32, i32]),
    "SetTextureParameter": (None, [u32, u32, i32]),
    "DeleteTexture": (None, [u32]),
    "DeleteRenderbuffer": (None, [u32]),
    "DeleteFramebuffer": (None, [u32]),
    "DeleteBuffer": (None, [u32]),
    "DeleteVertexArray": (None, [u32]),
    "DeleteQuery": (None, [u32]),
    "DeleteShader": (None, [u32]),
    "DeleteProgram": (None, [u32]),
    "LockFramebuffer": (P, [u32]),
    "LockTexture": (P, [u32]),
    "LockResource": (None, [P]),
    "UnlockResource": (None, [P]),
    "GetResourceBuffer": (P, [P, P, P, P]),
    "Composite": (None, [P, P, i32, i32, i32, i32, i32, i32, i32, i32, u8, u8, u8, u32, i32, i32, i32, i32]),
    "CompositeYUV": (None, [P, P, P, P, i32, u32, i32, i32, i32, i32, i32, i32, i32, i32, u8, u8, i32, i32, i32, i32]),
    "CreateContext": (P, []),
    "ReferenceContext": (None, [P]),
    "DestroyContext": (None, [P]),
    "MakeCurrent": (None, [P]),
    "ReportMemory": (usz, [P, P]),
}
assert len(SIGNATURES) == 99

EXTRA_SIGNATURES = {
    "WrhipGetStats": (None, [P]),
    "WrhipResetStats": (None, []),
    "WrhipSetProfiling": (None, [i32]),
    "WrhipGetKernelStats": (i32, [P, i32]),
    "WrhipSetShard": (None, [i32, i32]),
    "WrhipSetTargetRows": (None, [u32, i32, i32]),
    "WrhipGetTextureDevicePtr": (P, [u32, P, P, P]),
    "WrhipGetFramebufferTexture": (u32, [u32]),
    "WrhipDeviceName": (c_char_p, []),
    "WrhipFlush": (None, []),
    "WrhipFlushHeld": (i32, []),
    "WrhipGetStream": (P, []),
}


class WrhipStats(C.Structure):
    _fields_ = [(n, u64) for n in (
        "flushes", "kernel_launches", "raster_launches", "raster_ns",
        "raster_algo_bytes", "raster_pixels", "prims", "h2d_bytes", "d2h_bytes",
        "host_record_ns", "host_upload_ns", "host_flush_ns", "host_wait_ns", "row_launches",
        "setup_carried", "carrier_lost", "scratch_grown_held")]


class WrhipKernelStat(C.Structure):
    _fields_ = [(n, i32) for n in ("kind", "fmt", "depth", "feat")] + [(n, u64) for n in ("launches", "ns", "algo_bytes", "workgroups")]


def _as_ptr(x):
    if x is None:
        return None, None
    if isinstance(x, int):
        return x, None
    if isinstance(x, (bytes, bytearray)):
        buf = (C.c_char * len(x)).from_buffer_copy(x) if isinstance(x, bytes) \
            else (C.c_char * len(x)).from_buffer(x)
        return C.addressof(buf), buf
    if hasattr(x, "ctypes"):
        return x.ctypes.data, x
    return C.addressof(x), x


class GL:

    def __init__(self, path, trace=None):
        self.path = os.path.abspath(path)
        self._dll = C.CDLL(self.path, mode=os.RTLD_LOCAL | os.RTLD_NOW)
        self.trace = trace
        self.is_wrhip = hasattr(self._dll, "WrhipGetStats")
        for name, (res, args) in SIGNATURES.items():
            fn = getattr(self._dll, name)
            fn.restype, fn.argtypes = res, args
            setattr(self, name, self._wrap(name, fn, args))
        if self.is_wrhip:
            for name, (res, args) in EXTRA_SIGNATURES.items():
                fn = getattr(self._dll, name)
                fn.restype, fn.argtypes = res, args
                setattr(self, name, fn)

    def _wrap(self, name, fn, argtypes):
        ptr_idx = [i for i, t in enumerate(argtypes) if t is P]
        gl = self

        def call(*a):
            if gl.trace is not None and name == "GetUniformLocation":
                loc = fn(*a)
                gl.trace.record(name, a, ret=loc)
                return loc
            if gl.trace is not None:
                gl.trace.record(name, a)
            if ptr_idx:
                a = list(a)
                keep = []
                for i in ptr_idx:
                    a[i], k = _as_ptr(a[i])
                    keep.append(k)
            return fn(*a)
        call.__name__ = name
        return call

    def gen(self, fn_name):
        out = u32(0)
        getattr(self, fn_name)(1, out)
        return out.value

    def stats(self):
        s = WrhipStats()
        self.WrhipGetStats(C.byref(s))
        return {n: getattr(s, n) for n, _ in s._fields_}


def repo_root():
    return os.path.dirname(os.path.dirname(os.path.abspath(__file__)))


def wrhip_path():
    return os.environ.get("WRHIP_LIB_PATH") or os.path.join(repo_root(), "webrender_amd", "csrc", "libwrhip.so")


def load_wrhip(trace=None):
    p = wrhip_path()
    if not os.path.exists(p):
        raise RuntimeError(
            f"{p} not built -- run `python -c 'import __graft_entry__ as g; g.build()'`")
    return GL(p, trace)
# ... 1 lines not shown
```

Baseline: 30730 frames/s.

## Add specialized rect-only fused setup+raster kernel for simple draw batches

Adds a templated SIMPLE path through setup (vertex prim, finish prim, setup body) that strips clip stashes, AA records, mask rows, gradient tables and most shader cases. It also adds a fused setup+raster kernel variant with tighter launch bounds. The host picks this kernel when the carrier batch is plain RGBA8 with no features and every draw is a clear or a simple non-quad draw. The aim is lower register pressure and higher occupancy in the fused launch, at the cost of extra kernel instantiations and a second code path that must stay in step with the general one.

Result: slower. 28460 frames/s (-7.4%).

```diff
diff --git a/include/wrhip.h b/include/wrhip.h
--- a/include/wrhip.h
+++ b/include/wrhip.h
@@ -203,6 +203,7 @@
   uint64_t setup_carried;
   uint64_t carrier_lost;
   uint64_t scratch_grown_held;
+  uint64_t setup_simple;
 } WrhipStats;
 void WrhipGetStats(WrhipStats* out);
 void WrhipResetStats(void);
diff --git a/webrender_amd/csrc/wrhip.hip b/webrender_amd/csrc/wrhip.hip
--- a/webrender_amd/csrc/wrhip.hip
+++ b/webrender_amd/csrc/wrhip.hip
@@ -431,6 +431,7 @@
   std::vector<GLuint> view_texs;
   struct PendingScatter { size_t seg_off = 0; int nseg = 0, parts = 0; uint64_t bytes = 0; bool valid = false; } ps;
   bool fuse_scatter = true;
+  bool simple_setup = true;
   uint8_t* dupload = nullptr;
   struct Scratch {
     WrPrim* prims = nullptr; size_t prims_cap = 0;
@@ -519,6 +520,7 @@
       chain_grid = getenv("WRHIP_CHAIN_GRID") ? atoi(getenv("WRHIP_CHAIN_GRID")) : wrrt::cu_count() / 2;
     cell_raster = getenv("WRHIP_NO_CELLS") == nullptr;
     fuse_scatter = getenv("WRHIP_NO_FUSE_SCATTER") == nullptr;
+    simple_setup = getenv("WRHIP_NO_SIMPLE_SETUP") == nullptr;
     mask_rows = getenv("WRHIP_NO_MASK_ROWS") == nullptr;
     span_rows = getenv("WRHIP_NO_SPAN_ROWS") == nullptr;
     tile_rows = getenv("WRHIP_NO_TILE_ROWS") == nullptr;
@@ -1112,11 +1114,14 @@
   return H.fmt == WR_FMT_RGBA8 && (H.feat == 0 || H.feat == (WR_FEAT_TEX | WR_FEAT_GENERIC) ||
                                    H.feat == (WR_FEAT_TEX | WR_FEAT_GENERIC | WR_FEAT_R8TEX));
 }
+bool simple_carrier(const Context::Held& H) {
+  return H.row_n == 0 && H.mr_rows == 0 && !H.dense && H.fmt == WR_FMT_RGBA8 && H.feat == 0;
+}
 bool chainable(const Context::Held& H) {
   return ctx->chain_grid > 0 && H.row_n == 0 && H.fmt == WR_FMT_R8 && H.nb <= WR_THIN_MAX_BINS && (H.feat == 0 || H.feat == (WR_FEAT_GENERIC | WR_FEAT_BLUR));
 }
 void launch_raster(const Context::Held& H, const WrTargetDesc* targets, int n_targets, const WrDrawDesc* draws, Context::Scratch& S,
-                   const WrSetupArgs* SA = nullptr, int n_setup_blocks = 0, int chain_n = 1, uint64_t setup_bytes = 0) {
+                   const WrSetupArgs* SA = nullptr, int n_setup_blocks = 0, int chain_n = 1, uint64_t setup_bytes = 0, bool simple_setup = false) {
   Context* c = ctx;
 #define WR_K(FMT, DEPTH, FEAT)                                                                                          \
   do {                                                                                                                  \
@@ -1126,6 +1131,12 @@
 #define WR_KF(DEPTH, FEAT)                                                                                              \
   do {                                                                                                                  \
     WR_LAUNCH((wr_setup_raster_kernel<WR_FMT_RGBA8, DEPTH, 4, FEAT>), n_setup_blocks + SA->up_blocks + H.nb, 256, c->stream, *SA,        \
+              n_setup_blocks, targets, n_targets, draws, (const WrPrim*)S.prims, (const WrRec*)S.recs,                  \
+              (const WrAux*)S.aux, (const float*)S.vtab, S.masks, H.off);                                               \
+  } while (0)
+#define WR_KFS(DEPTH)                                                                                                   \
+  do {                                                                                                                  \
+    WR_LAUNCH((wr_setup_simple_raster_kernel<WR_FMT_RGBA8, DEPTH, 4, 0>), n_setup_blocks + SA->up_blocks + H.nb, 256, c->stream, *SA, \
               n_setup_blocks, targets, n_targets, draws, (const WrPrim*)S.prims, (const WrRec*)S.recs,                  \
               (const WrAux*)S.aux, (const float*)S.vtab, S.masks, H.off);                                               \
   } while (0)
@@ -1211,6 +1222,9 @@
     WR_LAUNCH((wr_setup_raster_thin_kernel<WR_FMT_RGBA8, false, 1, WR_FEAT_TEX | WR_FEAT_GENERIC>), n_setup_blocks + SA->up_blocks + H.nb * 4, 256, c->stream, *SA,
               n_setup_blocks, targets, n_targets, draws, (const WrPrim*)S.prims, (const WrRec*)S.recs, (const WrAux*)S.aux, (const float*)S.vtab, S.masks, H.off);
   }
+  else if (SA && simple_setup && H.feat == 0) {
+    if (H.depth) WR_KFS(true); else WR_KFS(false);
+  }
   else if (SA) {
     if (H.depth) {
       if (H.feat == 0) WR_KF(true, 0); else if (H.feat == F5) WR_KF(true, WR_FEAT_TEX | WR_FEAT_GENERIC);
@@ -1255,18 +1269,19 @@
   }
 #undef WR_K
 #undef WR_KF
+#undef WR_KFS
   prof_end(thin_wgs ? (fused ? 13 : 12) : fused ? (H.dense ? 7 : 6) : (H.dense ? 5 : 2), H.fmt, H.depth, H.feat, H.algo_bytes + (fused ? setup_bytes : 0),
            thin_wgs ? thin_wgs : (uint64_t)H.nb + (fused ? n_setup_blocks : 0));
   c->stats.kernel_launches++; c->stats.raster_launches++;
 }
 void launch_held(const std::vector<Context::Held>& held, const WrTargetDesc* targets, int n_targets, const WrDrawDesc* draws, Context::Scratch& S,
-                 int fuse_at = -1, const WrSetupArgs* SA = nullptr, int n_setup_blocks = 0, uint64_t setup_bytes = 0) {
+                 int fuse_at = -1, const WrSetupArgs* SA = nullptr, int n_setup_blocks = 0, uint64_t setup_bytes = 0, bool simple_setup = false) {
   for (size_t i = 0; i < held.size();) {
     size_t j = i + 1;
     if (chainable(held[i]) && !(S.mr_ctl == nullptr && held[i].mr_rows > 0))
       while (j < held.size() && j - i < WR_MAX_CHAIN && chainable(held[j]) && held[j].feat == held[i].feat && held[j].mr_rows == 0 && (int)j != fuse_at) j++;
     const bool fuse = (int)i == fuse_at;
-    launch_raster(held[i], targets, n_targets, draws, S, fuse ? SA : nullptr, fuse ? n_setup_blocks : 0, (int)(j - i), fuse ? setup_bytes : 0);
+    launch_raster(held[i], targets, n_targets, draws, S, fuse ? SA : nullptr, fuse ? n_setup_blocks : 0, (int)(j - i), fuse ? setup_bytes : 0, fuse && simple_setup);
     i = j;
   }
 }
@@ -1776,6 +1791,12 @@
       }
       for (size_t hi = 0; hi < c->tail.held.size() && fuse_at < 0; hi++) if (can_fuse(c->tail.held[hi])) fuse_at = (int)hi;
     }
+    bool simple_setup = false;
+    if (fuse_at >= 0 && c->simple_setup && simple_carrier(c->tail.held[fuse_at])) {
+      simple_setup = true;
+      for (int i = 0; i < nd && simple_setup; i++)
+        simple_setup = draws[i].shader == WR_SH_CLEAR_OP || ((draws[i].flags & WR_DF_SIMPLE) && !(draws[i].flags & WR_DF_QUADS));
+    }
     lap(1);
     flush_uploads(0, fuse_at >= 0);
     uint8_t* darena = c->dupload + aoff;
@@ -1825,7 +1846,8 @@
           c->ps.valid = false;
         }
         c->stats.setup_carried++;
-        launch_held(T.held, T.targets, T.n_targets, T.draws, c->scratch[T.set], fuse_at, &SA, n_setup_blocks, carried);
+        if (simple_setup) c->stats.setup_simple++;
+        launch_held(T.held, T.targets, T.n_targets, T.draws, c->scratch[T.set], fuse_at, &SA, n_setup_blocks, carried, simple_setup);
         tail_launched();
       } else {
         launch_pending_scatter();
diff --git a/webrender_amd/csrc/wrhip_inst.h b/webrender_amd/csrc/wrhip_inst.h
--- a/webrender_amd/csrc/wrhip_inst.h
+++ b/webrender_amd/csrc/wrhip_inst.h
@@ -19,5 +19,6 @@
   X(wr_raster_kernel, WR_SIG_PLAIN, WR_FMT_R8, false, 4, 28)
 #define WR_INST_7(X) X(wr_raster_kernel, WR_SIG_PLAIN, WR_FMT_RGBA8, false, 1, 5) X(wr_raster_kernel, WR_SIG_PLAIN, WR_FMT_RGBA8, false, 1, 47)
 #define WR_INST_8(X) X(wr_setup_raster_thin_kernel, WR_SIG_FUSED, WR_FMT_RGBA8, false, 1, 5)
-#define WR_INST_ALL(X) WR_INST_1(X) WR_INST_2(X) WR_INST_3(X) WR_INST_4(X) WR_INST_5(X) WR_INST_6(X) WR_INST_7(X) WR_INST_8(X)
-#define WR_INST_GROUPS 8
+#define WR_INST_9(X) X(wr_setup_simple_raster_kernel, WR_SIG_FUSED, WR_FMT_RGBA8, true, 4, 0) X(wr_setup_simple_raster_kernel, WR_SIG_FUSED, WR_FMT_RGBA8, false, 4, 0)
+#define WR_INST_ALL(X) WR_INST_1(X) WR_INST_2(X) WR_INST_3(X) WR_INST_4(X) WR_INST_5(X) WR_INST_6(X) WR_INST_7(X) WR_INST_8(X) WR_INST_9(X)
+#define WR_INST_GROUPS 9
diff --git a/webrender_amd/csrc/wrhip_k_raster.h b/webrender_amd/csrc/wrhip_k_raster.h
--- a/webrender_amd/csrc/wrhip_k_raster.h
+++ b/webrender_amd/csrc/wrhip_k_raster.h
@@ -1716,6 +1716,35 @@
   WR_FUSED_PROLOGUE(S, n_setup_blocks)
   wr_raster_body<FMT, DEPTH, R, FEAT>(targets, n_targets, draws, prims, recs, aux, vtab, masks, wr_bid + bin_offset);
 }
+#ifdef WRHIP_HOSTSIM
+#define WR_FUSED_SIMPLE_BOUNDS(DEPTH) __launch_bounds__(256)
+#else
+#ifndef WR_SIMPLE_WAVES
+#define WR_SIMPLE_WAVES 5
+#endif
+#define WR_FUSED_SIMPLE_BOUNDS(DEPTH) __launch_bounds__(256, (DEPTH) ? 4 : WR_SIMPLE_WAVES)
+#endif
+template <int FMT, bool DEPTH, int R, int FEAT>
+__global__ void WR_FUSED_SIMPLE_BOUNDS(DEPTH)
+wr_setup_simple_raster_kernel(WrSetupArgs S, int n_setup_blocks,
+                              const WrTargetDesc* __restrict__ targets, int n_targets,
+                              const WrDrawDesc* __restrict__ draws, const WrPrim* __restrict__ prims,
+                              const WrRec* __restrict__ recs, const WrAux* __restrict__ aux, const float* __restrict__ vtab,
+                              unsigned long long* __restrict__ masks, int bin_offset) {
+  static_assert(R == 4 && FMT == WR_FMT_RGBA8 && FEAT == 0, "the rect-only bin launch");
+  int wr_bid = (int)blockIdx.x;
+  if (wr_bid < S.up_blocks) { wr_upload_body(S.up_segs, S.up_nseg, S.up_parts, wr_bid); return; }
+  wr_bid -= S.up_blocks;
+  if (wr_bid < n_setup_blocks) {
+#ifndef WRHIP_HOSTSIM
+    __builtin_amdgcn_s_setprio(3);
+#endif
+    wr_setup_simple_body(S.draws, S.n_draws, S.arena, S.prims, S.recs, S.n_prims, S.targets, S.masks, S.cnt, S.blk, wr_bid);
+    return;
+  }
+  wr_bid -= n_setup_blocks;
+  wr_raster_body<FMT, DEPTH, R, FEAT>(targets, n_targets, draws, prims, recs, aux, vtab, masks, wr_bid + bin_offset);
+}
 template <int FMT, bool DEPTH, int R, int FEAT>
 __global__ void __launch_bounds__(256, WR_TEX_WAVES)
 wr_setup_raster_thin_kernel(WrSetupArgs S, int n_setup_blocks,
diff --git a/webrender_amd/csrc/wrhip_k_setup.h b/webrender_amd/csrc/wrhip_k_setup.h
--- a/webrender_amd/csrc/wrhip_k_setup.h
+++ b/webrender_amd/csrc/wrhip_k_setup.h
@@ -2510,6 +2510,7 @@
   for (int i = 0; i < bytes / 4; i++) d[i] = s[i];
 }
 
+template <bool SIMPLE = false>
 WR_DEVICE void wr_finish_prim(const WrDrawDesc& d, int draw_index, const WrVsOut& o, WrPrim& P, WrAux* auxp,
                               WrUnsupportedCounters* cnt) {
   P.kind = WR_PK_NONE;
@@ -2535,7 +2536,7 @@
                                                                               d.shader == WR_SH_PS_QUAD_RADIAL_GRADIENT || d.shader == WR_SH_PS_QUAD_CONIC_GRADIENT));
     if (!(o.kind == WR_PK_SOLID || ptex)) { atomicAdd(&cnt->perspective_prims, 1u); return; }
     clipped = !inside;
-    if (clipped) {
+    if (!SIMPLE && clipped) {
       WrClipStash& St = *wr_clip_stash(auxp->quad);
       for (int n = 0; n < 4; n++) { St.px[n] = o.px[n]; St.py[n] = o.py[n]; St.pz[n] = o.pz[n]; St.pw[n] = o.pw[n]; St.u[n] = o.u[n]; St.v[n] = o.v[n]; }
       St.two = o.kind == WR_PK_MIX_BLEND ? 1 : 0;
@@ -2602,6 +2603,10 @@
   bool typeA = sy[0] == sy[1] && sy[2] == sy[3] && sx[0] == sx[3] && sx[1] == sx[2];
   bool typeB = sx[0] == sx[1] && sx[2] == sx[3] && sy[0] == sy[3] && sy[1] == sy[2];
   if ((!typeA && !typeB) || (aa && texq) || persp) {
+    if constexpr (SIMPLE) {
+      if (persp) { atomicAdd(&cnt->perspective_prims, 1u); return; }
+      P.kind = WR_PK_UNSUPPORTED; atomicAdd(&cnt->unsupported_prims, 1u); return;
+    } else {
     const bool solidq = o.kind == WR_PK_SOLID && !masked && !(d.flags & WR_DF_SIMPLE);
     if (persp && !solidq && !(texq && (o.kind == WR_PK_TEX_RGBA8 || o.kind == WR_PK_TEX_FS || o.kind == WR_PK_TEX_R8 || o.kind == WR_PK_TEX_REPEAT || o.kind == WR_PK_FILTER || o.kind == WR_PK_GRADIENT || o.kind == WR_PK_QUAD_MASK || (o.kind == WR_PK_SOLID && masked) || o.kind == WR_PK_MIX_BLEND || o.kind == WR_PK_YUV))) {
       atomicAdd(&cnt->perspective_prims, 1u); return;
@@ -2666,6 +2671,7 @@
     P.fcolor[0] = o.color.x; P.fcolor[1] = o.color.y; P.fcolor[2] = o.color.z; P.fcolor[3] = o.color.w;
     if (o.blend_override != 0 && d.blend != WR_BLEND_NONE) { P.blend = (int16_t)o.blend_override; wr_pack_color(o.blend_color, P.color); }
     return;
+    }
   }
   float xa = sx[0], xb = sx[2], ya = sy[0], yb = sy[2];
   float xmin = wr_min(xa, xb), xmax = wr_max(xa, xb), ymin = wr_min(ya, yb), ymax = wr_max(ya, yb);
@@ -2681,11 +2687,13 @@
     const int l_end = ml ? int(ceilf(sx0)) : int(floorf(sx0 + 0.5f));
     const int r_end = mr ? int(ceilf(sx1)) : int(floorf(sx1 + 0.5f));
     ix0 = l_start; ix1 = r_end;
+    if constexpr (!SIMPLE) {
     WrAARec& A = auxp->aa;
     const float dxl = (-1.0f * 256.0f) * (1.0f / sqrtf(1.0f + 0.0f * 0.0f)), dxr = (1.0f * 256.0f) * (1.0f / sqrtf(1.0f + 0.0f * 0.0f));
     A.lstart = ml ? 128.0f + dxl * (xmin - 0.5f) : 256.0f; A.lend = ml ? -dxl : 0.0f;
     A.rstart = mr ? 128.0f + dxr * (xmax - 0.5f) : 256.0f; A.rend = mr ? -dxr : 0.0f;
     A.laa_end = l_end;
+    }
     aaRound = 0.0f;
   }
   float ystart = floorf(wr_max(wr_min(ymin, cy1), cy0) + aaRound) + 0.5f;
@@ -2700,12 +2708,12 @@
   P.kind = (masked && o.kind == WR_PK_SOLID) ? (int16_t)WR_PK_SOLID_MASKED : (aa ? (int16_t)WR_PK_SOLID_AA : (int16_t)o.kind);
   if (masked && o.kind != WR_PK_SOLID) P.flags |= WR_PF_MASKED;
   P.rows_linear = 0;
-  if ((d.flags & WR_DF_SIMPLE) && P.kind != WR_PK_SOLID) {
+  if ((SIMPLE || (d.flags & WR_DF_SIMPLE)) && P.kind != WR_PK_SOLID) {
     P.kind = WR_PK_UNSUPPORTED; atomicAdd(&cnt->unsupported_prims, 1u); return;
   }
   if (o.kind == WR_PK_UNSUPPORTED) { atomicAdd(&cnt->unsupported_prims, 1u); return; }
   const bool blend_override = o.blend_override != 0 && d.blend != WR_BLEND_NONE;
-  if (o.kind == WR_PK_SOLID) {
+  if (SIMPLE || o.kind == WR_PK_SOLID) {
     wr_pack_color(o.color, P.color);
     if (masked) P.tex_slot = WR_S_CLIP_MASK;
   } else if (o.kind == WR_PK_TEX_RGBA8 || o.kind == WR_PK_TEX_R8 || o.kind == WR_PK_BLUR || o.kind == WR_PK_TEX_FS || o.kind == WR_PK_CLIP_RECT || o.kind == WR_PK_BOX_SHADOW || o.kind == WR_PK_GRADIENT || o.kind == WR_PK_FILTER || o.kind == WR_PK_MIX_BLEND || o.kind == WR_PK_SVG_FILTER || o.kind == WR_PK_YUV || o.kind == WR_PK_QUAD_MASK || o.kind == WR_PK_TEX_REPEAT || o.kind == WR_PK_BORDER_SOLID || o.kind == WR_PK_BORDER_SEGMENT || o.kind == WR_PK_FAST_GRADIENT || o.kind == WR_PK_LINE_DECORATION) {
@@ -3848,6 +3856,7 @@
 __device__ unsigned long long wr_dbg_mid[16384];
 __device__ unsigned wr_dbg_prim[16384 * 4];
 #endif
+template <bool SIMPLE = false>
 WR_DEVICE void wr_vertex_prim(const WrDescView& V, int n_draws, const uint8_t* __restrict__ arena,
                               int gid, WrPrim& P, WrAux* aux, WrUnsupportedCounters* cnt) {
   P.blend = 0; P.flags = 0; P.z = 0; P.color[0] = P.color[1] = 0; P.tex_slot = 0;
@@ -3875,6 +3884,17 @@
   o.uv_add[0] = o.uv_add[1] = 0.0f;
   o.blend_override = 0; o.blend_color = wf4{0, 0, 0, 0}; o.persp_div = -1.0f; o.dual = 0; o.dual_swz = 0.0f;
   o.cd[0] = o.cd[1] = 0; o.cd[2] = o.cd[3] = -1;
+  if constexpr (SIMPLE) {
+    switch (d.shader) {
+      case WR_SH_PS_QUAD_TEXTURED: wr_vs_ps_quad_textured(d, arena, inst, o); break;
+      case WR_SH_BRUSH_SOLID:
+      case WR_SH_BRUSH_SOLID_ALPHA: wr_vs_brush(d, arena, inst, 0, o); break;
+      default:
+        P.kind = WR_PK_UNSUPPORTED; P.x0 = P.x1 = P.y0 = P.y1 = 0; P.draw = lo; atomicAdd(&cnt->unsupported_prims, 1u);
+        return;
+    }
+    wr_finish_prim<true>(d, lo, o, P, nullptr, cnt);
+  } else {
   switch (d.shader) {
     case WR_SH_PS_QUAD_TEXTURED: wr_vs_ps_quad_textured(d, arena, inst, o); break;
     case WR_SH_PS_QUAD_MASK: wr_vs_ps_quad_textured(d, arena, inst, o, 1, &aux[gid].clip); break;
@@ -3956,9 +3976,10 @@
       if (any) atomicMin(&fr[V.target(d.target).height], (uint32_t)gid);
     }
   }
+  }
   if (d.query_slot >= 0 && P.kind != WR_PK_NONE && P.kind != WR_PK_UNSUPPORTED) {
     unsigned long long n = 0;
-    if (P.kind == WR_PK_SOLID_QUAD || P.kind == WR_PK_TEX_QUAD) {
+    if (!SIMPLE && (P.kind == WR_PK_SOLID_QUAD || P.kind == WR_PK_TEX_QUAD)) {
       for (int y = P.y0; y < P.y1; y++) { int s0, s1; if (wr_quad_row_span(aux[gid].quad, y, s0, s1)) { s0 = wr_imax(s0, P.x0); s1 = wr_imin(s1, P.x1); if (s1 > s0) n += (unsigned long long)(s1 - s0); } }
     } else {
       n = (unsigned long long)(P.x1 - P.x0) * (unsigned long long)(P.y1 - P.y0);
@@ -4304,6 +4325,7 @@
   }
 }
 
+template <bool SIMPLE = false>
 WR_DEVICE void wr_setup_body(const WrDrawDesc* __restrict__ draws, int n_draws,
                                 const uint8_t* __restrict__ arena, WrPrim* __restrict__ prims,
                                 WrRec* __restrict__ recs, WrAux* __restrict__ aux, int n_prims,
@@ -4347,7 +4369,7 @@
 #endif
   }
   WR_TP(1);
-  if (valid) wr_vertex_prim(V, n_draws, arena, gid, P, aux, cnt);
+  if (valid) wr_vertex_prim<SIMPLE>(V, n_draws, arena, gid, P, aux, cnt);
   WR_TP(7);
 #ifdef WRHIP_TIMING
   const unsigned long long tm1 = wall_clock64();
@@ -4363,6 +4385,7 @@
     const WrRec rec_ = wr_make_rec(P, T_.format);
     recs[gid] = rec_;
     if (T_.rows_mode || ((rec_.kbf & 0xFF) != WR_PK_SOLID_FOLDED && (rec_.kbf & 0xFF) != WR_PK_NONE)) prims[gid] = P;
+    if constexpr (!SIMPLE) {
     if ((P.kind == WR_PK_BOX_SHADOW || P.kind == WR_PK_CLIP_RECT) && (D_.flags & WR_DF_MASK_ROWS) && P.x1 > P.x0 && P.y1 > P.y0) {
       const WrTargetDesc& T = T_;
       if (T.mr_ctl) {
@@ -4412,7 +4435,9 @@
         aux[gid].tex.simple = 0;
       }
     }
-  }
+    }
+  }
+  if constexpr (!SIMPLE) {
   int mr_slot = -1;
   wr_mask_rows_reserve(mr_T, mr_rows, mr_pitch, mr_n16, mr_tabs16, gid, V.draw(P.draw).target, recs, mr_slot);
   if (mr_slot >= 0) {
@@ -4435,6 +4460,7 @@
     else if (valid && P.kind == WR_PK_TEX_QUAD && aux[gid].quad.base_kind == WR_PK_GRADIENT) Gq = &aux[gid].quad.grad;
     wr_grad_tables_wave(V, P.draw, gid, Gq);
     if (Gq) wr_grad_merge_bits(Gq);
+  }
   }
 #ifdef WRHIP_TIMING
   const unsigned long long tm2 = wall_clock64();
@@ -4455,6 +4481,13 @@
 #endif
 }
 
+WR_DEVICE void wr_setup_simple_body(const WrDrawDesc* __restrict__ draws, int n_draws, const uint8_t* __restrict__ arena,
+                                    WrPrim* __restrict__ prims, WrRec* __restrict__ recs, int n_prims,
+                                    const WrTargetDesc* __restrict__ targets, unsigned long long* __restrict__ masks,
+                                    WrUnsupportedCounters* cnt, const int* __restrict__ blk, const int bid) {
+  wr_setup_body<true>(draws, n_draws, arena, prims, recs, nullptr, n_prims, targets, masks, nullptr, cnt, blk, bid);
+}
+
 #ifndef WR_INST_ONLY
 __global__ void __launch_bounds__(256, 3) wr_setup_kernel(const WrDrawDesc* __restrict__ draws, int n_draws,
                                 const uint8_t* __restrict__ arena, WrPrim* __restrict__ prims,
diff --git a/webrender_amd/glapi.py b/webrender_amd/glapi.py
--- a/webrender_amd/glapi.py
+++ b/webrender_amd/glapi.py
@@ -130,7 +130,7 @@
         "flushes", "kernel_launches", "raster_launches", "raster_ns",
         "raster_algo_bytes", "raster_pixels", "prims", "h2d_bytes", "d2h_bytes",
         "host_record_ns", "host_upload_ns", "host_flush_ns", "host_wait_ns", "row_launches",
-        "setup_carried", "carrier_lost", "scratch_grown_held")]
+        "setup_carried", "carrier_lost", "scratch_grown_held", "setup_simple")]
 
 
 class WrhipKernelStat(C.Structure):
```
